# timmywanttolearn/distributed_model_parallel

Measured on AMD Instinct MI355X. Metric: images/sec (whole node) ResNet-50 DDP bf16, higher is better.
Workload: dtype bf16; 1 GPU; model=resnet50, device=cuda, global_batch=2048, per_gpu_batch=2048, image_size=224, parallelism=ddp1, single_rank_comm=False, ranks=1, rccl_ranks=1, launcher=single, optimizer=FlatSGD(fp32 master), sync_bn=False, channels_last=True, grad_comm=none(world_size=1), hip_graph=False, checkpoint_segments=0

## Files before the change

### csrc/api.h

```cpp
#pragma once

#include <ATen/ATen.h>
#include <c10/util/Optional.h>

#include <cstdint>
#include <string>
#include <vector>

namespace dmp {

bool attention_supported(int64_t S, int64_t head_dim);
void set_attention_variant(int fwd, int bwd);
std::vector<int64_t> get_attention_variant();
void set_attention_long_from(int64_t n);
int64_t get_attention_long_from();
std::vector<at::Tensor> attention_forward(const at::Tensor& qkv, int64_t B, int64_t S, int64_t H, double scale);
at::Tensor attention_backward(const at::Tensor& dout, const at::Tensor& qkv, const at::Tensor& o,
                              const at::Tensor& lse, int64_t B, int64_t S, int64_t H, double scale);

at::Tensor bn_local_moments(const at::Tensor& x, int64_t C);
std::vector<at::Tensor> bn_forward_apply(const at::Tensor& x, const at::Tensor& sums,
                                         const c10::optional<at::Tensor>& weight,
                                         const c10::optional<at::Tensor>& bias,
                                         const c10::optional<at::Tensor>& running_mean,
                                         const c10::optional<at::Tensor>& running_var,
                                         double momentum, double eps,
                                         const c10::optional<at::Tensor>& residual, bool relu,
                                         int64_t C,
                                         const c10::optional<at::Tensor>& num_batches_tracked,
                                         bool out_moments, double clip);
std::vector<at::Tensor> bn_eval_apply(const at::Tensor& x, const at::Tensor& running_mean,
                                      const at::Tensor& running_var,
                                      const c10::optional<at::Tensor>& weight,
                                      const c10::optional<at::Tensor>& bias, double eps,
                                      const c10::optional<at::Tensor>& residual, bool relu,
                                      int64_t C, double clip);
at::Tensor bn_backward_moments(const at::Tensor& dy, const at::Tensor& x,
                               const c10::optional<at::Tensor>& y, const at::Tensor& mean,
                               bool relu, int64_t C, const c10::optional<at::Tensor>& weight,
                               const c10::optional<at::Tensor>& bias,
                               const c10::optional<at::Tensor>& invstd, double clip);
at::Tensor bn_finalize(const at::Tensor& sums, const c10::optional<at::Tensor>& weight,
                       const c10::optional<at::Tensor>& bias,
                       const c10::optional<at::Tensor>& running_mean,
                       const c10::optional<at::Tensor>& running_var, double momentum, double eps,
                       int64_t C, const c10::optional<at::Tensor>& num_batches_tracked);
std::vector<at::Tensor> bn_backward_apply(const at::Tensor& dy, const at::Tensor& x,
                                          const c10::optional<at::Tensor>& y,
                                          const at::Tensor& sums, const at::Tensor& count,
                                          const c10::optional<at::Tensor>& weight,
                                          const at::Tensor& mean, const at::Tensor& invstd,
                                          bool training, bool relu, bool want_dres, int64_t C,
                                          const c10::optional<at::Tensor>& bias, double clip,
                                          const c10::optional<at::Tensor>& acc_weight,
                                          const c10::optional<at::Tensor>& acc_bias);
void set_bn_streaming(bool on);

bool bn_apply_gram_supported(int64_t C);
std::vector<at::Tensor> bn_forward_apply_gram(const at::Tensor& x, const at::Tensor& sums,
                                              const c10::optional<at::Tensor>& weight,
                                              const c10::optional<at::Tensor>& bias,
                                              const c10::optional<at::Tensor>& running_mean,
                                              const c10::optional<at::Tensor>& running_var, double momentum,
                                              double eps, int64_t C,
                                              const c10::optional<at::Tensor>& num_batches_tracked, double clip);
void set_bn_gram_blocks(int64_t n);

bool bn_fold_supported(int64_t cout, int64_t cin);
std::vector<at::Tensor> bn_fold_fwd(const at::Tensor& W, const at::Tensor& G, const at::Tensor& asums,
                                    const c10::optional<at::Tensor>& Wf);
std::vector<at::Tensor> bn_fold_fwd_finalize(const at::Tensor& W, const at::Tensor& G, const at::Tensor& asums,
                                             const c10::optional<at::Tensor>& Wf,
                                             const c10::optional<at::Tensor>& weight,
                                             const c10::optional<at::Tensor>& bias,
                                             const c10::optional<at::Tensor>& running_mean,
                                             const c10::optional<at::Tensor>& running_var, double momentum,
                                             double eps, const c10::optional<at::Tensor>& num_batches_tracked);
at::Tensor bn_fold_bwd_sums(const at::Tensor& D, const at::Tensor& W, const at::Tensor& sdz,
                            const at::Tensor& mean);
std::vector<at::Tensor> bn_fold_bwd_coef(const at::Tensor& sums, const at::Tensor& local, const at::Tensor& count,
                                         const at::Tensor& invstd, const at::Tensor& mean,
                                         const c10::optional<at::Tensor>& gamma, const at::Tensor& D,
                                         const at::Tensor& WG, const at::Tensor& s, const at::Tensor& W);
std::vector<at::Tensor> bn_fold_relu_mask(const at::Tensor& dy, const at::Tensor& y);
at::Tensor bn_fold_colsum(const at::Tensor& x, const std::vector<int64_t>& map);
std::vector<at::Tensor> bn_fold_scale_concat(const at::Tensor& W3, const at::Tensor& s3, const at::Tensor& t3,
                                             const at::Tensor& Wd, const at::Tensor& sd, const at::Tensor& td);
void set_fold_gemm(int mode);
int get_fold_gemm();

void multi_copy(const std::vector<at::Tensor>& srcs, const std::vector<at::Tensor>& dsts);
void multi_transpose(const std::vector<at::Tensor>& srcs, const std::vector<at::Tensor>& dsts,
                     const std::vector<int64_t>& taps);
void multi_cast_bf16_f32(const std::vector<at::Tensor>& srcs, const std::vector<at::Tensor>& dsts);
void reduce_add_into(const std::vector<at::Tensor>& inputs, at::Tensor& out);
void gather_slabs(const std::vector<at::Tensor>& inputs, at::Tensor& out, bool along_inner);
std::vector<std::vector<bool>> enable_peer_access(int64_t num_devices);

std::vector<at::Tensor> conv3x3_c128(const at::Tensor& x, const at::Tensor& wmat, bool moments);
bool conv3x3_c128_supported(int64_t c, int64_t h, int64_t w);
at::Tensor conv3x3_c128_dgrad_s2(const at::Tensor& dy, const at::Tensor& wt);

std::vector<at::Tensor> conv3x3_c64(const at::Tensor& x, const at::Tensor& wmat, bool moments);

std::vector<at::Tensor> dwconv3x3_forward(const at::Tensor& x, const at::Tensor& w, int64_t stride,
                                          bool moments);
at::Tensor dwconv3x3_dgrad(const at::Tensor& dy, const at::Tensor& w, int64_t stride, int64_t H,
                           int64_t W);
at::Tensor dwconv3x3_wgrad(const at::Tensor& dy, const at::Tensor& x, int64_t stride,
                           at::ScalarType out_dtype, const c10::optional<at::Tensor>& out);

std::vector<at::Tensor> gemm_nt(const at::Tensor& A, const at::Tensor& B,
                                const c10::optional<at::Tensor>& pro_scale,
                                const c10::optional<at::Tensor>& pro_shift, const std::string& mode,
                                const c10::optional<at::Tensor>& epi_scale,
                                const c10::optional<at::Tensor>& epi_shift,
                                const c10::optional<at::Tensor>& residual, bool relu,
                                const std::vector<int64_t>& a_map,
                                const std::vector<int64_t>& c_map,
                                const c10::optional<at::Tensor>& a2,
                                const std::vector<int64_t>& a2_map);
std::vector<at::Tensor> gemm_nt_bnbwd(const at::Tensor& A, const at::Tensor& B,
                                      const c10::optional<at::Tensor>& residual,
                                      const c10::optional<at::Tensor>& bn_x,
                                      const c10::optional<at::Tensor>& bn_y,
                                      const c10::optional<at::Tensor>& mean,
                                      const c10::optional<at::Tensor>& invstd,
                                      const c10::optional<at::Tensor>& weight,
                                      const c10::optional<at::Tensor>& bias,
                                      const std::vector<int64_t>& res_map,
                                      const c10::optional<at::Tensor>& a2,
                                      const c10::optional<at::Tensor>& ebias,
                                      const std::vector<int64_t>& a2_map);
at::Tensor gemm_tn(const at::Tensor& A, const at::Tensor& B, at::ScalarType out_dtype,
                   const std::vector<int64_t>& b_map, const c10::optional<at::Tensor>& pro_scale,
                   const c10::optional<at::Tensor>& pro_shift, bool a_mapped,
                   const c10::optional<at::Tensor>& out);
std::vector<at::Tensor> conv_nt(const at::Tensor& x, const at::Tensor& wmat, int64_t kh,
                                int64_t kw, int64_t stride, int64_t pad, int64_t ho, int64_t wo,
                                bool transposed, const c10::optional<at::Tensor>& pro_scale,
                                const c10::optional<at::Tensor>& pro_shift,
                                const std::string& mode,
                                const c10::optional<at::Tensor>& epi_scale,
                                const c10::optional<at::Tensor>& epi_shift,
                                const c10::optional<at::Tensor>& residual, bool relu,
                                int64_t kc);
at::Tensor conv_wgrad(const at::Tensor& dy, const at::Tensor& x, int64_t kh, int64_t kw,
                      int64_t stride, int64_t pad, int64_t ho, int64_t wo,
                      at::ScalarType out_dtype, int64_t kc, const c10::optional<at::Tensor>& out);
void set_gemm_tile(int64_t t);
void set_phase_dgrad(bool on);
void set_tn_wide(bool on);

at::Tensor space_to_depth2(const at::Tensor& x, int64_t pad, int64_t out_channels);
at::Tensor pad_channels16(const at::Tensor& x, int64_t pad, int64_t extra_w);

bool stem_halo_supported(int64_t hs, int64_t ws, int64_t ho, int64_t wo);
std::vector<at::Tensor> stem_halo_fwd(const at::Tensor& s, const at::Tensor& wm, int64_t ho, bool moments);
at::Tensor stem_halo_wgrad(const at::Tensor& dy, const at::Tensor& s, int64_t ho, at::ScalarType out_dtype);
std::vector<at::Tensor> stem_halo_wgrad_pool(const at::Tensor& dy, const at::Tensor& idx, const at::Tensor& y,
                                             const at::Tensor& s, const at::Tensor& scale, const at::Tensor& shift,
                                             const at::Tensor& mean, int64_t ho, int64_t pad);
at::Tensor stem_fold_finish(const at::Tensor& img, int64_t ho, int64_t wo, const at::Tensor& t_dz,
                            const at::Tensor& t_y, const at::Tensor& sums, const at::Tensor& cnt,
                            const at::Tensor& invstd, const c10::optional<at::Tensor>& weight, const at::Tensor& mean,
                            at::ScalarType out_dtype);

at::Tensor wgrad3x3(const at::Tensor& dy, const at::Tensor& x, int64_t stride);
bool wgrad3x3_supported(int64_t C, int64_t H, int64_t W, int64_t stride);
void set_wgrad3x3_waves(int64_t nw);

at::Tensor augment_batch(const at::Tensor& src, const at::Tensor& plan, int64_t out_h, int64_t out_w,
                         const std::vector<double>& mean, const std::vector<double>& std_, at::ScalarType dtype,
                         bool channels_last, bool no_resize);

at::Tensor batch_mix(const at::Tensor& x, const at::Tensor& perm, double lam, const std::vector<int64_t>& box);

at::Tensor gemm_xl(const at::Tensor& A, const at::Tensor& B, const std::string& mode,
                   const c10::optional<at::Tensor>& bias, const c10::optional<at::Tensor>& aux,
                   const c10::optional<at::Tensor>& residual, const c10::optional<at::Tensor>& out,
                   const c10::optional<at::Tensor>& row_scale = c10::nullopt, int64_t rows_per_sample = 0);
std::vector<at::Tensor> gemm_xl_dgelu_bgrad(const at::Tensor& A, const at::Tensor& B, const at::Tensor& aux);
std::vector<at::Tensor> gemm_xl_conv(const at::Tensor& A, const at::Tensor& B, const std::string& mode,
                                     const c10::optional<at::Tensor>& residual,
                                     const c10::optional<at::Tensor>& bn_x,
                                     const c10::optional<at::Tensor>& bn_y,
                                     const c10::optional<at::Tensor>& mean,
                                     const c10::optional<at::Tensor>& invstd,
                                     const c10::optional<at::Tensor>& weight,
                                     const c10::optional<at::Tensor>& bias,
                                     const std::vector<int64_t>& res_map,
                                     const c10::optional<at::Tensor>& a2,
                                     const c10::optional<at::Tensor>& ebias,
                                     const c10::optional<at::Tensor>& scale,
                                     const c10::optional<at::Tensor>& shift, bool relu,
                                     const std::vector<int64_t>& a2_map);
std::vector<at::Tensor> conv_xl(const at::Tensor& x, const at::Tensor& wmat, int64_t kh, int64_t kw,
                                int64_t stride, int64_t pad, int64_t ho, int64_t wo, const std::string& mode,
                                const c10::optional<at::Tensor>& residual, const c10::optional<at::Tensor>& bn_x,
                                const c10::optional<at::Tensor>& bn_y, const c10::optional<at::Tensor>& mean,
                                const c10::optional<at::Tensor>& invstd, const c10::optional<at::Tensor>& weight,
                                const c10::optional<at::Tensor>& bias);
at::Tensor conv_xl_dgrad_s2(const at::Tensor& dy, const std::vector<at::Tensor>& wph, int64_t hi, int64_t wi);
void set_gemm_xl_bn(int bn, int pipe, int group_m);
int get_gemm_xl_pipe();
void set_gemm_xl_x2(int mode);
int get_gemm_xl_x2();
void set_gemm_xl_bm(int bm);
int get_gemm_xl_bm(int64_t M, int64_t N, int64_t K);
void set_gemm_xl_trace(const c10::optional<at::Tensor>& buf);
void set_gemm_xl_trim_heavy(bool on);

at::Tensor gemm_tn_xl(const at::Tensor& A, const at::Tensor& B, at::ScalarType out_dtype,
                      const c10::optional<at::Tensor>& out);
at::Tensor gram_strided_xl(const at::Tensor& x, int64_t stride, int64_t ho, int64_t wo);
bool gram_strided_xl_supported(int64_t nb, int64_t cin, int64_t hi, int64_t wi, int64_t ho, int64_t wo);
at::Tensor conv_wgrad_xl(const at::Tensor& dy, const at::Tensor& x, int64_t kh, int64_t kw, int64_t stride,
                         int64_t pad, int64_t ho, int64_t wo, at::ScalarType out_dtype,
                         const c10::optional<at::Tensor>& out);
void set_tn_xl_rounds(int r);
void set_tn_narrow(bool on);

bool colsum_supported(int64_t N);
at::Tensor bias_grad(const at::Tensor& dy, at::ScalarType out_dtype);
std::vector<at::Tensor> gelu_bwd_bias_grad(const at::Tensor& dy, const at::Tensor& h, at::ScalarType out_dtype);
std::vector<at::Tensor> rowscale_bias_grad(const at::Tensor& dy, const at::Tensor& row_scale, int64_t rows_per_sample,
                                           at::ScalarType out_dtype);

std::vector<at::Tensor> cross_entropy_fwd(const at::Tensor& x, const at::Tensor& target,
                                          int64_t ignore_index, double scale,
                                          const c10::optional<at::Tensor>& acc, double label_smoothing,
                                          const c10::optional<at::Tensor>& target_b, double lam);
at::Tensor cross_entropy_bwd(const at::Tensor& grad, const at::Tensor& x, const at::Tensor& target,
                             const at::Tensor& lse, const at::Tensor& stats, int64_t ignore_index,
                             double label_smoothing, const c10::optional<at::Tensor>& target_b, double lam);
std::vector<at::Tensor> layernorm_forward(const at::Tensor& x, const c10::optional<at::Tensor>& w,
                                          const c10::optional<at::Tensor>& b, int64_t D,
                                          double eps);
std::vector<at::Tensor> layernorm_backward(const at::Tensor& dy, const at::Tensor& x,
                                           const c10::optional<at::Tensor>& w,
                                           const at::Tensor& mean, const at::Tensor& rstd,
                                           int64_t D, at::ScalarType param_dtype,
                                           const c10::optional<at::Tensor>& dres);
bool layernorm_supported(int64_t D);

void flat_sumsq_partials(const at::Tensor& grad, at::Tensor& partials_row);
void adamw_prepare(const c10::optional<at::Tensor>& partials, at::Tensor& hyper, at::Tensor& step,
                   double max_norm, double beta1, double beta2);
void adamw_flat_step(const c10::optional<at::Tensor>& master, at::Tensor& exp_avg, at::Tensor& exp_avg_sq,
                     const at::Tensor& grad, at::Tensor& param,
                     const c10::optional<at::Tensor>& decay_mask, const at::Tensor& hyper, double lr,
                     double beta1, double beta2, double eps, double weight_decay,
                     const c10::optional<at::Tensor>& ema, double ema_decay);
int64_t adamw_grid_cap();

void lars_norm_partials(const c10::optional<at::Tensor>& master, const at::Tensor& grad,
                        const at::Tensor& param, const at::Tensor& items, at::Tensor& partials);
void lars_trust(const at::Tensor& partials, const at::Tensor& tensors, at::Tensor& coef,
                double trust_coefficient, double weight_decay, double eps);
void lars_flat_step(const c10::optional<at::Tensor>& master, at::Tensor& mom, const at::Tensor& grad,
                    at::Tensor& param, const at::Tensor& items, const at::Tensor& coef, double lr,
                    double momentum, const c10::optional<at::Tensor>& ema, double ema_decay);
int64_t lars_chunk_elems();
int64_t lars_fold_threads();

void sgd_flat_step(const c10::optional<at::Tensor>& master, const at::Tensor& mom,
                   const at::Tensor& grad, const at::Tensor& param, double lr, double wd,
                   double momentum, double dampening, bool nesterov, double grad_scale,
                   bool first_step, const c10::optional<at::Tensor>& ema, double ema_decay);

std::vector<at::Tensor> maxpool2d_forward(const at::Tensor& x, int64_t k, int64_t s, int64_t p);
at::Tensor maxpool2d_backward(const at::Tensor& dy, const at::Tensor& idx, int64_t H, int64_t W,
                              int64_t k, int64_t s, int64_t p);
at::Tensor global_avgpool_backward(const at::Tensor& g, int64_t H, int64_t W);
std::vector<at::Tensor> maxpool2d_bn_forward(const at::Tensor& x, const at::Tensor& scale,
                                             const at::Tensor& shift, int64_t k, int64_t s, int64_t p);
std::vector<at::Tensor> maxpool2d_bn_backward(const at::Tensor& dy, const at::Tensor& idx, const at::Tensor& x,
                                              const at::Tensor& scale, const at::Tensor& shift,
                                              const at::Tensor& mean, int64_t k, int64_t s, int64_t p);
void set_pool_generic(bool on);

}
```

### csrc/bindings.cpp

```cpp
#include <cmath>
#include <torch/extension.h>
#include <torch/csrc/autograd/variable.h>

#include "api.h"
#include "comm/rccl_comm.h"
#include "ddp/reducer.h"
#include "dp/parallel_apply.h"

namespace py = pybind11;

PYBIND11_MODULE(TORCH_EXTENSION_NAME, m) {
  m.doc() = "MI355X-native runtime: RCCL communicator, DDP reducer, HIP kernels (gfx950)";

  m.def("bn_local_moments", &dmp::bn_local_moments,
        py::call_guard<py::gil_scoped_release>());
  m.def("bn_forward_apply", &dmp::bn_forward_apply, py::arg("x"), py::arg("sums"), py::arg("weight"),
        py::arg("bias"), py::arg("running_mean"), py::arg("running_var"), py::arg("momentum"),
        py::arg("eps"), py::arg("residual"), py::arg("relu"), py::arg("C"),
        py::arg("num_batches_tracked") = py::none(), py::arg("out_moments") = false,
        py::arg("clip") = INFINITY,
        py::call_guard<py::gil_scoped_release>());
  m.def("bn_forward_apply_gram", &dmp::bn_forward_apply_gram, py::arg("x"), py::arg("sums"), py::arg("weight"),
        py::arg("bias"), py::arg("running_mean"), py::arg("running_var"), py::arg("momentum"), py::arg("eps"),
        py::arg("C"), py::arg("num_batches_tracked") = py::none(), py::arg("clip") = INFINITY,
        "training-mode BN + ReLU apply that also returns the column moments and the fp32 Gram of its output",
        py::call_guard<py::gil_scoped_release>());
  m.def("bn_apply_gram_supported", &dmp::bn_apply_gram_supported);
  m.def("set_bn_gram_blocks", &dmp::set_bn_gram_blocks);
  m.def("bn_eval_apply", &dmp::bn_eval_apply, py::arg("x"), py::arg("running_mean"),
        py::arg("running_var"), py::arg("weight"), py::arg("bias"), py::arg("eps"), py::arg("residual"),
        py::arg("relu"), py::arg("C"), py::arg("clip") = INFINITY,
        py::call_guard<py::gil_scoped_release>());
  m.def("bn_finalize", &dmp::bn_finalize, py::arg("sums"), py::arg("weight"), py::arg("bias"),
        py::arg("running_mean"), py::arg("running_var"), py::arg("momentum"), py::arg("eps"),
        py::arg("C"), py::arg("num_batches_tracked") = py::none(),
        py::call_guard<py::gil_scoped_release>());
  m.def("bn_backward_moments", &dmp::bn_backward_moments, py::arg("dy"), py::arg("x"), py::arg("y"),
        py::arg("mean"), py::arg("relu"), py::arg("C"), py::arg("weight") = py::none(),
        py::arg("bias") = py::none(), py::arg("invstd") = py::none(), py::arg("clip") = INFINITY,
        py::call_guard<py::gil_scoped_release>());
  m.def("bn_backward_apply", &dmp::bn_backward_apply, py::arg("dy"), py::arg("x"), py::arg("y"),
        py::arg("sums"), py::arg("count"), py::arg("weight"), py::arg("mean"), py::arg("invstd"),
        py::arg("training"), py::arg("relu"), py::arg("want_dres"), py::arg("C"),
        py::arg("bias") = py::none(), py::arg("clip") = INFINITY, py::arg("acc_weight") = py::none(),
        py::arg("acc_bias") = py::none(),
        py::call_guard<py::gil_scoped_release>());

  m.def("gemm_nt", &dmp::gemm_nt, py::arg("A"), py::arg("B"), py::arg("pro_scale") = py::none(),
        py::arg("pro_shift") = py::none(), py::arg("mode") = "store",
        py::arg("epi_scale") = py::none(), py::arg("epi_shift") = py::none(),
        py::arg("residual") = py::none(), py::arg("relu") = false,
        py::arg("a_map") = std::vector<int64_t>{}, py::arg("c_map") = std::vector<int64_t>{},
        py::arg("a2") = py::none(), py::arg("a2_map") = std::vector<int64_t>{},
        py::call_guard<py::gil_scoped_release>());

  m.def("cross_entropy_fwd", &dmp::cross_entropy_fwd, py::arg("x"), py::arg("target"),
        py::arg("ignore_index") = -100, py::arg("scale") = 1.0, py::arg("acc") = py::none(),
        py::arg("label_smoothing") = 0.0, py::arg("target_b") = py::none(), py::arg("lam") = 1.0,
        "scale * mean softmax cross-entropy; acc (fp64 [3]) += (loss, top-1 correct, top-5 correct); "
        "label_smoothing and a second label target_b weighted 1 - lam give the soft-target loss",
        py::call_guard<py::gil_scoped_release>());
  m.def("cross_entropy_bwd", &dmp::cross_entropy_bwd, py::arg("grad"), py::arg("x"), py::arg("target"),
        py::arg("lse"), py::arg("stats"), py::arg("ignore_index") = -100, py::arg("label_smoothing") = 0.0,
        py::arg("target_b") = py::none(), py::arg("lam") = 1.0, py::call_guard<py::gil_scoped_release>());
  m.def("batch_mix", &dmp::batch_mix, py::arg("x"), py::arg("perm"), py::arg("lam"),
        py::arg("box") = std::vector<int64_t>{},
        "mixup (empty box): lam * x[i] + (1 - lam) * x[perm[i]]; CutMix (box = [y0, y1, x0, x1]): "
        "x[perm[i]] inside the box, x[i] outside; channels-last bf16 / fp32, out of place",
        py::call_guard<py::gil_scoped_release>());
  m.def("augment_batch", &dmp::augment_batch, py::arg("src"), py::arg("plan"), py::arg("out_h"), py::arg("out_w"),
        py::arg("mean"), py::arg("std"), py::arg("dtype"), py::arg("channels_last") = true, py::arg("no_resize") = false,
        "uint8 NHWC batch -> [B, C, out_h, out_w] bf16 / fp32: per-sample crop box plan[i] = (x0, y0, cw, ch, flip) "
        "(zero padding outside the image, bilinear resize when the box is not out_h x out_w), flip, /255, "
        "mean / std normalisation, cast and layout in one launch; no_resize: every box is out_h x out_w (the crop-only kernel; "
        "other rows come out NaN)",
        py::call_guard<py::gil_scoped_release>());
  m.def("gemm_nt_bnbwd", &dmp::gemm_nt_bnbwd, py::arg("A"), py::arg("B"), py::arg("residual"),
        py::arg("bn_x"), py::arg("bn_y"), py::arg("mean"), py::arg("invstd"), py::arg("weight"),
        py::arg("bias"), py::arg("res_map") = std::vector<int64_t>{}, py::arg("a2") = py::none(),
        py::arg("ebias") = py::none(), py::arg("a2_map") = std::vector<int64_t>{},
        py::call_guard<py::gil_scoped_release>());

  m.def("gemm_tn", &dmp::gemm_tn, py::arg("A"), py::arg("B"), py::arg("out_dtype"),
        py::arg("b_map") = std::vector<int64_t>{}, py::arg("pro_scale") = py::none(),
        py::arg("pro_shift") = py::none(), py::arg("a_mapped") = false, py::arg("out") = py::none(),
        "C = A^T B (weight gradient); b_map reads B's rows through a strided map, a_mapped A's too (Gram of a "
        "sample); out: add into this gradient instead of returning a new tensor",
        py::call_guard<py::gil_scoped_release>());

  m.def("set_tn_wide", &dmp::set_tn_wide, py::arg("on"),
        "128 x 256 TN tiles for deep weight gradients (default on)");
  m.def("set_phase_dgrad", &dmp::set_phase_dgrad, py::arg("on"),
        "strided implicit-GEMM data gradients as stride-phase launches (default on)");
  m.def("set_gemm_tile", &dmp::set_gemm_tile,
        "debug: force the NT GEMM tile variant (-1 auto, 0 256x64, 1 128x64, 2 128x128, "
        "3 128x64/4x1, 4 64x128, 5 64x64)");

  m.def("conv_nt", &dmp::conv_nt, py::arg("x"), py::arg("wmat"), py::arg("kh"), py::arg("kw"),
        py::arg("stride"), py::arg("pad"), py::arg("ho"), py::arg("wo"),
        py::arg("transposed") = false, py::arg("pro_scale") = py::none(),
        py::arg("pro_shift") = py::none(), py::arg("mode") = "store",
        py::arg("epi_scale") = py::none(), py::arg("epi_shift") = py::none(),
        py::arg("residual") = py::none(), py::arg("relu") = false, py::arg("kc") = 0,
        py::call_guard<py::gil_scoped_release>());
  m.def("conv_wgrad", &dmp::conv_wgrad, py::arg("dy"), py::arg("x"), py::arg("kh"), py::arg("kw"),
        py::arg("stride"), py::arg("pad"), py::arg("ho"), py::arg("wo"), py::arg("out_dtype"),
        py::arg("kc") = 0, py::arg("out") = py::none(),
        py::call_guard<py::gil_scoped_release>());
  m.def("maxpool2d_bn_forward", &dmp::maxpool2d_bn_forward, py::arg("x"), py::arg("scale"),
        py::arg("shift"), py::arg("k"), py::arg("s"), py::arg("p"),
        py::call_guard<py::gil_scoped_release>());
  m.def("maxpool2d_bn_backward", &dmp::maxpool2d_bn_backward, py::arg("dy"), py::arg("idx"), py::arg("x"),
        py::arg("scale"), py::arg("shift"), py::arg("mean"), py::arg("k"), py::arg("s"), py::arg("p"),
        py::call_guard<py::gil_scoped_release>());
  m.def("pad_channels16", &dmp::pad_channels16, py::arg("x"), py::arg("pad"), py::arg("extra_w") = 0,
        py::call_guard<py::gil_scoped_release>());
  m.def("space_to_depth2", &dmp::space_to_depth2, py::arg("x"), py::arg("pad"), py::arg("out_channels") = 16,
        py::call_guard<py::gil_scoped_release>());

  m.def("gemm_xl", &dmp::gemm_xl, py::arg("A"), py::arg("B"), py::arg("mode") = "store",
        py::arg("bias") = py::none(), py::arg("aux") = py::none(),
        py::arg("residual") = py::none(), py::arg("out") = py::none(), py::kw_only(),
        py::arg("row_scale") = py::none(), py::arg("rows_per_sample") = 0,
        py::call_guard<py::gil_scoped_release>());
  m.def("conv_xl", &dmp::conv_xl, py::arg("x"), py::arg("wmat"), py::arg("kh"), py::arg("kw"),
        py::arg("stride"), py::arg("pad"), py::arg("ho"), py::arg("wo"), py::arg("mode") = "moments",
        py::arg("residual") = py::none(), py::arg("bn_x") = py::none(), py::arg("bn_y") = py::none(),
        py::arg("mean") = py::none(), py::arg("invstd") = py::none(), py::arg("weight") = py::none(),
        py::arg("bias") = py::none(),
        "Implicit-GEMM conv (NHWC gather) on the 256x256 ping-pong MFMA kernel with conv epilogues",
        py::call_guard<py::gil_scoped_release>());
  m.def("stem_halo_supported", &dmp::stem_halo_supported);
  m.def("stem_halo_fwd", &dmp::stem_halo_fwd, py::arg("s"), py::arg("wm"), py::arg("ho"), py::arg("moments") = false,
        "ResNet stem (s2d 4x4 conv, 16 -> 64 ch, Wo = 112) forward: halo-tiled, weights in VGPRs",
        py::call_guard<py::gil_scoped_release>());
  m.def("stem_fold_finish", &dmp::stem_fold_finish, py::arg("img"), py::arg("ho"), py::arg("wo"), py::arg("t_dz"),
        py::arg("t_y"), py::arg("sums"), py::arg("cnt"), py::arg("invstd"), py::arg("weight"), py::arg("mean"),
        py::arg("out_dtype"),
        "folded stem weight gradient: BN-backward coefficients, the 16 window sums of the batch-summed "
        "space-to-depth image, and al t_dz + be t_y + cc cols in one launch",
        py::call_guard<py::gil_scoped_release>());
  m.def("stem_halo_wgrad", &dmp::stem_halo_wgrad, py::arg("dy"), py::arg("s"), py::arg("ho"), py::arg("out_dtype"),
        "ResNet stem weight gradient [64, 256]: halo-tiled, dW in VGPRs",
        py::call_guard<py::gil_scoped_release>());
  m.def("stem_halo_wgrad_pool", &dmp::stem_halo_wgrad_pool, py::arg("dy"), py::arg("idx"), py::arg("y"), py::arg("s"),
        py::arg("scale"), py::arg("shift"), py::arg("mean"), py::arg("ho"), py::arg("pad"),
        "ResNet stem folded backward: (dz^T P, y^T P, BN-backward sums) with the pool / ReLU backward formed in LDS",
        py::call_guard<py::gil_scoped_release>());
  m.def("wgrad3x3", &dmp::wgrad3x3, py::arg("dy"), py::arg("x"), py::arg("stride") = 1,
        "dW [C, C, 3, 3] (channels_last) of a 3x3/s1/p1 conv: persistent halo-tiled MFMA kernel",
        py::call_guard<py::gil_scoped_release>());
  m.def("wgrad3x3_supported", &dmp::wgrad3x3_supported, py::arg("C"), py::arg("Ho"), py::arg("Wo"),
        py::arg("stride") = 1);
  m.def("set_wgrad3x3_waves", &dmp::set_wgrad3x3_waves);
  m.def("conv3x3_c64", &dmp::conv3x3_c64, py::arg("x"), py::arg("wmat"), py::arg("moments") = false,
        "3x3/s1/p1 64->64-channel conv (W = 56) on the persistent halo-tiled MFMA kernel; "
        "returns (y [N*H*W, 64], fp64 moments [129] or empty)",
        py::call_guard<py::gil_scoped_release>());
  m.def("conv3x3_c128", &dmp::conv3x3_c128, py::arg("x"), py::arg("wmat"), py::arg("moments") = false,
        "3x3/s1/p1 128->128-channel conv (W = 28, H % 4 == 0) on the persistent halo-tiled MFMA kernel "
        "(Cout split over grid halves, K split over wave pairs); returns (y [N*H*W, 128], fp64 moments [257] or empty)",
        py::call_guard<py::gil_scoped_release>());
  m.def("conv3x3_c128_dgrad_s2", &dmp::conv3x3_c128_dgrad_s2, py::arg("dy"), py::arg("wt"),
        "data gradient of a 3x3/s2/p1 128->128 conv (dy 28 wide) as its four stride phases on the halo kernel; "
        "wt = W.permute(1, 2, 3, 0) as [128, 1152]; returns dx [N*2H*56, 128]",
        py::call_guard<py::gil_scoped_release>());
  m.def("conv3x3_c128_supported", &dmp::conv3x3_c128_supported, py::arg("C"), py::arg("H"), py::arg("W"));
  m.def("conv_xl_dgrad_s2", &dmp::conv_xl_dgrad_s2, py::arg("dy"), py::arg("wph"), py::arg("hi"), py::arg("wi"),
        "data gradient of a 3x3/s2/p1 conv as four stride-phase implicit GEMMs on the ping-pong kernel; "
        "returns dx [N*hi*wi, Cin]",
        py::call_guard<py::gil_scoped_release>());
  m.def("set_bn_streaming", &dmp::set_bn_streaming, py::arg("on"),
        "A/B: non-temporal streaming in the BN apply passes over > 256 MB tensors (default on)");
  m.def("set_pool_generic", &dmp::set_pool_generic, py::arg("on"),
        "A/B: route every max-pool geometry through the runtime-k kernels (default off)");
  m.def("set_tn_xl_rounds", &dmp::set_tn_xl_rounds, py::arg("rounds"));
  m.def("set_gemm_xl_trim_heavy", &dmp::set_gemm_xl_trim_heavy, py::arg("on"),
        "A/B: trimmed (192..240-row) tiles for the PIPE-10 heavy-epilogue GEMMs at any K (default on)");
  m.def("set_tn_narrow", &dmp::set_tn_narrow, py::arg("on"),
        "A/B: 4-wave weight-gradient tiles of 64 / 128 on an output side that narrow (default on)");
  m.def("gemm_tn_xl", &dmp::gemm_tn_xl, py::arg("A"), py::arg("B"), py::arg("out_dtype"), py::arg("out") = py::none(),
        "A^T B (weight gradient) on the ping-pong MFMA schedule, split over M",
        py::call_guard<py::gil_scoped_release>());
  m.def("gram_strided_xl", &dmp::gram_strided_xl, py::arg("x"), py::arg("stride"), py::arg("ho"), py::arg("wo"),
        "fp32 Gram x_s^T x_s of the stride-s sample of an NHWC bf16 input (4-wave TN kernel, both operands gathered)",
        py::call_guard<py::gil_scoped_release>());
  m.def("gram_strided_xl_supported", &dmp::gram_strided_xl_supported);
  m.def("conv_wgrad_xl", &dmp::conv_wgrad_xl, py::arg("dy"), py::arg("x"), py::arg("kh"), py::arg("kw"),
        py::arg("stride"), py::arg("pad"), py::arg("ho"), py::arg("wo"), py::arg("out_dtype"),
        py::arg("out") = py::none(),
        "kh x kw conv weight gradient (tap gather) on the ping-pong TN kernel; Cin % 256 == 0",
        py::call_guard<py::gil_scoped_release>());
  m.def("gemm_xl_dgelu_bgrad", &dmp::gemm_xl_dgelu_bgrad, py::arg("A"), py::arg("B"), py::arg("aux"),
        py::call_guard<py::gil_scoped_release>());
  m.def("gemm_xl_conv", &dmp::gemm_xl_conv, py::arg("A"), py::arg("B"), py::arg("mode"),
        py::arg("residual") = py::none(), py::arg("bn_x") = py::none(), py::arg("bn_y") = py::none(),
        py::arg("mean") = py::none(), py::arg("invstd") = py::none(), py::arg("weight") = py::none(),
        py::arg("bias") = py::none(), py::arg("res_map") = std::vector<int64_t>{},
        py::arg("a2") = py::none(), py::arg("ebias") = py::none(), py::arg("scale") = py::none(),
        py::arg("shift") = py::none(), py::arg("relu") = false, py::arg("a2_map") = std::vector<int64_t>{},
        "wide 1x1-conv GEMM with conv epilogues: moments | add | bnbwd | affine (scale, shift, residual, relu); "
        "a2: second A source concatenated along K; ebias: bnbwd per-column constant",
        py::call_guard<py::gil_scoped_release>());
  m.def("get_gemm_xl_pipe", &dmp::get_gemm_xl_pipe);
  m.def("set_gemm_xl_x2", &dmp::set_gemm_xl_x2, py::arg("mode"),
        "conv-epilogue GEMMs on the two-blocks-per-CU 256x128 kernel: 0 off, 1 where N % 256 != 0, 2 always");
  m.def("get_gemm_xl_x2", &dmp::get_gemm_xl_x2);
  m.def("set_gemm_xl_bm", &dmp::set_gemm_xl_bm, py::arg("bm"),
        "256x256 ping-pong GEMMs: rows per tile (0 auto: trimmed to fill whole rounds when K >= 768; "
        "-1 always 256; 192..240 forced)");
  m.def("set_gemm_xl_trace", &dmp::set_gemm_xl_trace, py::arg("buf") = py::none(),
        "diagnostics: 256x256 ping-pong GEMM launches record per-block phase timestamps into buf "
        "(int64 [blocks * 8]: entry, operands landed, main loop done, epilogue done, HW_ID, XCC_ID); None = off");
  m.def("get_gemm_xl_bm", &dmp::get_gemm_xl_bm, py::arg("M"), py::arg("N"), py::arg("K"),
        "rows per tile the ping-pong GEMM would take for this shape");
  m.def("set_gemm_xl_bn", &dmp::set_gemm_xl_bn, py::arg("bn"), py::arg("pipe") = -1, py::arg("group_m") = 0,
        "debug: force the gemm_xl N tile (0 auto, 128, 256) and main loop (0, 1, 10, 11; -1 default)");

  m.def("bn_fold_supported", &dmp::bn_fold_supported, py::arg("cout"), py::arg("cin"));
  m.def("bn_fold_fwd_finalize", &dmp::bn_fold_fwd_finalize, py::arg("W"), py::arg("G"), py::arg("asums"),
        py::arg("Wf"), py::arg("weight"), py::arg("bias"), py::arg("running_mean"), py::arg("running_var"),
        py::arg("momentum"), py::arg("eps"), py::arg("num_batches_tracked"),
        "bn_fold_fwd + the BN finalize of its moments in one launch: (sums, WG, coef[4, Cout])");
  m.def("bn_fold_fwd", &dmp::bn_fold_fwd, py::arg("W"), py::arg("G"), py::arg("asums"), py::arg("Wf") = py::none(),
        "(sums fp64 [2Cout+1], WG fp32 [Cout, Cin]) of y = a W^T from G = a^T a and colsum(a)",
        py::call_guard<py::gil_scoped_release>());
  m.def("bn_fold_bwd_sums", &dmp::bn_fold_bwd_sums, py::arg("D"), py::arg("W"), py::arg("sdz"), py::arg("mean"),
        "local fp64 [2Cout] = (sum dz, sum dz*(y - mean)) from D = dz^T a",
        py::call_guard<py::gil_scoped_release>());
  m.def("bn_fold_bwd_coef", &dmp::bn_fold_bwd_coef, py::arg("sums"), py::arg("local"), py::arg("count"),
        py::arg("invstd"), py::arg("mean"), py::arg("gamma"), py::arg("D"), py::arg("WG"), py::arg("s"),
        py::arg("W"), "(dW, dgamma, dbeta, Bm = [(al o W)^T | W^T diag(be) W], ebias = c^T W)",
        py::call_guard<py::gil_scoped_release>());

  m.def("bn_fold_relu_mask", &dmp::bn_fold_relu_mask, py::arg("dy"), py::arg("y"),
        py::call_guard<py::gil_scoped_release>());
  m.def("bn_fold_colsum", &dmp::bn_fold_colsum, py::arg("x"), py::arg("map") = std::vector<int64_t>{},
        "fp64 [2C+1] (colsum, colsum of squares, rows) of x's rows sampled through a strided map",
        py::call_guard<py::gil_scoped_release>());
  m.def("bn_fold_scale_concat", &dmp::bn_fold_scale_concat, py::arg("W3"), py::arg("s3"), py::arg("t3"),
        py::arg("Wd"), py::arg("sd"), py::arg("td"), "([s3 o W3 | sd o Wd] bf16, t3 + td)",
        py::call_guard<py::gil_scoped_release>());

  m.def("attention_supported", &dmp::attention_supported);
  m.def("set_fold_gemm", &dmp::set_fold_gemm, py::arg("mode"),
        "BN-fold coefficient products: 0 fused VALU kernels, 1 library fp32 GEMMs (default), 2 tiled kernel");
  m.def("get_fold_gemm", &dmp::get_fold_gemm);
  m.def("get_attention_variant", &dmp::get_attention_variant);
  m.def("set_attention_variant", &dmp::set_attention_variant, py::arg("fwd"), py::arg("bwd") = 1,
        "attention kernels: fwd 0 = one workgroup per (batch, head), 1 = persistent with next-head prefetch, "
        "2 = 8-wave per head; bwd 0 = per head, 1 = persistent with prefetch.  Selects among the S <= 256 "
        "kernels only: the streamed long-sequence kernels (set_attention_long_from) have one variant each");
  m.def("get_attention_long_from", &dmp::get_attention_long_from);
  m.def("set_attention_long_from", &dmp::set_attention_long_from, py::arg("n"),
        "sequences of n tokens or more run the streamed long-sequence attention kernels (default 257: "
        "everything the whole-sequence-in-LDS kernels cannot hold; 1 = always, for A/B runs and tests)");
  m.def("attention_forward", &dmp::attention_forward, py::arg("qkv"), py::arg("B"), py::arg("S"),
        py::arg("H"), py::arg("scale"),
        py::call_guard<py::gil_scoped_release>());
  m.def("attention_backward", &dmp::attention_backward, py::arg("dout"), py::arg("qkv"), py::arg("o"),
        py::arg("lse"), py::arg("B"), py::arg("S"), py::arg("H"), py::arg("scale"),
        py::call_guard<py::gil_scoped_release>());

  m.def("colsum_supported", &dmp::colsum_supported);
  m.def("bias_grad", &dmp::bias_grad, py::arg("dy"), py::arg("out_dtype"),
        py::call_guard<py::gil_scoped_release>());
  m.def("gelu_bwd_bias_grad", &dmp::gelu_bwd_bias_grad, py::arg("dy"), py::arg("h"), py::arg("out_dtype"),
        py::call_guard<py::gil_scoped_release>());
  m.def("rowscale_bias_grad", &dmp::rowscale_bias_grad, py::arg("dy"), py::arg("row_scale"),
        py::arg("rows_per_sample"), py::arg("out_dtype"), py::call_guard<py::gil_scoped_release>());

  m.def("layernorm_forward", &dmp::layernorm_forward,
        py::call_guard<py::gil_scoped_release>());
  m.def("layernorm_backward", &dmp::layernorm_backward, py::arg("dy"), py::arg("x"), py::arg("w"),
        py::arg("mean"), py::arg("rstd"), py::arg("D"), py::arg("param_dtype"),
        py::arg("dres") = py::none(),
        py::call_guard<py::gil_scoped_release>());
  m.def("layernorm_supported", &dmp::layernorm_supported);

  m.def("maxpool2d_forward", &dmp::maxpool2d_forward,
        py::call_guard<py::gil_scoped_release>());
  m.def("maxpool2d_backward", &dmp::maxpool2d_backward,
        py::call_guard<py::gil_scoped_release>());
  m.def("global_avgpool_backward", &dmp::global_avgpool_backward,
        py::call_guard<py::gil_scoped_release>());

  m.def("dwconv3x3_forward", &dmp::dwconv3x3_forward, py::arg("x"), py::arg("w"),
        py::arg("stride"), py::arg("moments") = false,
        py::call_guard<py::gil_scoped_release>());
  m.def("dwconv3x3_dgrad", &dmp::dwconv3x3_dgrad,
        py::call_guard<py::gil_scoped_release>());
  m.def("dwconv3x3_wgrad", &dmp::dwconv3x3_wgrad, py::arg("dy"), py::arg("x"), py::arg("stride"),
        py::arg("out_dtype"), py::arg("out") = py::none(),
        py::call_guard<py::gil_scoped_release>());

  m.def("sgd_flat_step", &dmp::sgd_flat_step, py::arg("master"), py::arg("mom"), py::arg("grad"),
        py::arg("param"), py::arg("lr"), py::arg("wd"), py::arg("momentum"), py::arg("dampening"),
        py::arg("nesterov"), py::arg("grad_scale"), py::arg("first_step"), py::arg("ema") = py::none(),
        py::arg("ema_decay") = 0.0,
        py::call_guard<py::gil_scoped_release>());
  m.def("flat_sumsq_partials", &dmp::flat_sumsq_partials, py::arg("grad"), py::arg("partials_row"),
        "partials_row[b] = block b's sum of squares of the flat gradient (fixed order, no atomics)",
        py::call_guard<py::gil_scoped_release>());
  m.def("adamw_prepare", &dmp::adamw_prepare, py::arg("partials"), py::arg("hyper"), py::arg("step"),
        py::arg("max_norm"), py::arg("beta1"), py::arg("beta2"),
        "step += 1; hyper = {1 - beta1^step, 1 - beta2^step, gradient norm, clip coefficient}",
        py::call_guard<py::gil_scoped_release>());
  m.def("adamw_flat_step", &dmp::adamw_flat_step, py::arg("master"), py::arg("exp_avg"),
        py::arg("exp_avg_sq"), py::arg("grad"), py::arg("param"), py::arg("decay_mask"), py::arg("hyper"),
        py::arg("lr"), py::arg("beta1"), py::arg("beta2"), py::arg("eps"), py::arg("weight_decay"),
        py::arg("ema") = py::none(), py::arg("ema_decay") = 0.0,
        py::call_guard<py::gil_scoped_release>());
  m.def("adamw_grid_cap", &dmp::adamw_grid_cap);
  m.def("lars_norm_partials", &dmp::lars_norm_partials, py::arg("master"), py::arg("grad"), py::arg("param"),
        py::arg("items"), py::arg("partials"),
        "partials[i] = {sum g^2, sum w^2} over work item i (fixed order, no atomics)",
        py::call_guard<py::gil_scoped_release>());
  m.def("lars_trust", &dmp::lars_trust, py::arg("partials"), py::arg("tensors"), py::arg("coef"),
        py::arg("trust_coefficient"), py::arg("weight_decay"), py::arg("eps"),
        "coef[t] = {trust ratio, weight decay, |w|, |g|} of tensor t; {1, 0, ..} for an excluded tensor",
        py::call_guard<py::gil_scoped_release>());
  m.def("lars_flat_step", &dmp::lars_flat_step, py::arg("master"), py::arg("mom"), py::arg("grad"),
        py::arg("param"), py::arg("items"), py::arg("coef"), py::arg("lr"), py::arg("momentum"),
        py::arg("ema") = py::none(), py::arg("ema_decay") = 0.0,
        py::call_guard<py::gil_scoped_release>());
  m.def("lars_chunk_elems", &dmp::lars_chunk_elems);
  m.def("lars_fold_threads", &dmp::lars_fold_threads);

  m.def("multi_copy", &dmp::multi_copy,
        py::call_guard<py::gil_scoped_release>());
  m.def("multi_cast_bf16_f32", &dmp::multi_cast_bf16_f32, py::arg("srcs"), py::arg("dsts"),
        "dst[i] (fp32) = src[i] (bf16) for contiguous tensors, up to 64 per launch",
        py::call_guard<py::gil_scoped_release>());
  m.def("multi_transpose", &dmp::multi_transpose, py::arg("srcs"), py::arg("dsts"),
        py::arg("taps") = std::vector<int64_t>{},
        "dst[i] = src[i]^T for contiguous 2-byte matrices, up to 64 per launch; taps[i] = T (-T: "
        "flipped) transposes [R, T*C] -> [C, T*R] tap by tap",
        py::call_guard<py::gil_scoped_release>());
  m.def("reduce_add_into", &dmp::reduce_add_into,
        py::call_guard<py::gil_scoped_release>());
  m.def("gather_slabs", &dmp::gather_slabs,
        py::call_guard<py::gil_scoped_release>());
  m.def("enable_peer_access", &dmp::enable_peer_access);

  py::class_<dmp::RcclComm, std::shared_ptr<dmp::RcclComm>>(m, "RcclComm")
      .def(py::init<const std::string&, int64_t, int64_t, int64_t, bool>(), py::arg("unique_id"),
           py::arg("nranks"), py::arg("rank"), py::arg("device"), py::arg("high_priority") = false,
           py::call_guard<py::gil_scoped_release>())
      .def("set_inline", &dmp::RcclComm::set_inline)
      .def("is_inline", &dmp::RcclComm::is_inline)
      .def_static("new_unique_id", [] { return py::bytes(dmp::RcclComm::new_unique_id()); })
      .def_property_readonly("rank", &dmp::RcclComm::rank)
      .def_property_readonly("size", &dmp::RcclComm::size)
      .def_property_readonly("device", &dmp::RcclComm::device)
      .def("all_reduce", &dmp::RcclComm::all_reduce, py::arg("tensor"), py::arg("op") = "sum",
           py::arg("on_current_stream") = false, py::call_guard<py::gil_scoped_release>())
      .def("all_reduce_coalesced", &dmp::RcclComm::all_reduce_coalesced, py::arg("tensors"),
           py::arg("op") = "sum", py::call_guard<py::gil_scoped_release>())
      .def("broadcast", &dmp::RcclComm::broadcast, py::call_guard<py::gil_scoped_release>())
      .def("reduce", &dmp::RcclComm::reduce, py::arg("tensor"), py::arg("root"),
           py::arg("op") = "sum", py::call_guard<py::gil_scoped_release>())
      .def("all_gather", &dmp::RcclComm::all_gather, py::call_guard<py::gil_scoped_release>())
      .def("reduce_scatter", &dmp::RcclComm::reduce_scatter, py::arg("out"), py::arg("inp"),
           py::arg("op") = "sum", py::call_guard<py::gil_scoped_release>())
      .def("all_to_all", &dmp::RcclComm::all_to_all, py::call_guard<py::gil_scoped_release>())
      .def("send", &dmp::RcclComm::send, py::call_guard<py::gil_scoped_release>())
      .def("recv", &dmp::RcclComm::recv, py::call_guard<py::gil_scoped_release>())
      .def("batch_p2p", &dmp::RcclComm::batch_p2p, py::call_guard<py::gil_scoped_release>())
      .def("wait", &dmp::RcclComm::wait, py::call_guard<py::gil_scoped_release>())
      .def("synchronize", &dmp::RcclComm::synchronize, py::call_guard<py::gil_scoped_release>())
      .def("stream_handle",
           [](const dmp::RcclComm& c) { return reinterpret_cast<uintptr_t>(c.stream()); });

  py::class_<dmp::ParallelApply, std::shared_ptr<dmp::ParallelApply>>(m, "ParallelApply")
      .def(py::init<>())
      .def("apply", &dmp::ParallelApply::apply, py::arg("modules"), py::arg("inputs"),
           py::arg("kwargs"), py::arg("devices"), py::arg("streams") = std::vector<int64_t>{})
      .def("num_workers", &dmp::ParallelApply::num_workers)
      .def("last_times", &dmp::ParallelApply::last_times);

  py::class_<dmp::ReduceBackend, std::shared_ptr<dmp::ReduceBackend>>(m, "ReduceBackend");
  py::class_<dmp::RcclReduceBackend, dmp::ReduceBackend, std::shared_ptr<dmp::RcclReduceBackend>>(
      m, "RcclReduceBackend")
      .def(py::init<std::shared_ptr<dmp::RcclComm>, double, int64_t, bool>(), py::arg("comm"),
           py::arg("postscale") = 1.0, py::arg("debug_delay_cycles") = 0, py::arg("fp32_accum") = false)
      .def("set_timing", &dmp::RcclReduceBackend::set_timing, py::arg("on"))
      .def("last_timing", &dmp::RcclReduceBackend::last_timing,
           "[ready->done ms per bucket..., collective ms per bucket..., exposed tail ms] of the last backward",
           py::call_guard<py::gil_scoped_release>());
  py::class_<dmp::NullReduceBackend, dmp::ReduceBackend, std::shared_ptr<dmp::NullReduceBackend>>(
      m, "NullReduceBackend")
      .def(py::init<>());
  py::class_<dmp::PyReduceBackend, dmp::ReduceBackend, std::shared_ptr<dmp::PyReduceBackend>>(
      m, "PyReduceBackend")
      .def(py::init<py::object>());

  py::class_<dmp::Reducer, std::shared_ptr<dmp::Reducer>>(m, "Reducer")
      .def(py::init<std::vector<at::Tensor>, std::vector<std::vector<int64_t>>,
                    std::shared_ptr<dmp::ReduceBackend>, bool>(),
           py::arg("params"), py::arg("buckets"), py::arg("backend"), py::arg("find_unused"))
      .def("prepare_for_backward", &dmp::Reducer::prepare_for_backward,
           py::call_guard<py::gil_scoped_release>())
      .def("disarm", &dmp::Reducer::disarm)
      .def("rebuild", &dmp::Reducer::rebuild, py::call_guard<py::gil_scoped_release>())
      .def("buckets", &dmp::Reducer::buckets)
      .def("ready_order", &dmp::Reducer::ready_order)
      .def("group_flats", &dmp::Reducer::group_flats)
      .def("layout", &dmp::Reducer::layout)
      .def("grad_views", &dmp::Reducer::grad_views)
      .def("unused_params", &dmp::Reducer::unused_params)
      .def("num_launched", &dmp::Reducer::num_launched)
      .def("set_backend", &dmp::Reducer::set_backend)
      .def("zero_grad", &dmp::Reducer::zero_grad, py::call_guard<py::gil_scoped_release>());

  m.def("compute_bucket_assignment", &dmp::compute_bucket_assignment, py::arg("params"),
        py::arg("cap_bytes"), py::arg("first_cap_bytes"));
  m.def("grad_accumulator_stream", [](const at::Tensor& t) -> int64_t {
    auto acc = torch::autograd::impl::try_get_grad_accumulator(t);
    if (!acc) return -1;
    auto s = acc->stream();
    return s.has_value() ? (int64_t)s->id() : -2;
  });
}
```

### csrc/conv/conv3x3_c128.hip

```cpp
#include <torch/extension.h>
#include <ATen/hip/HIPContext.h>
#include "../api.h"
#include "../common.h"
#include "../launch.h"

namespace dmp {
namespace {

using bf16 = __bf16;
using lptr_t = __attribute__((address_space(3))) void*;

constexpr int CI = 128, CO = 128, CB = 64;
constexpr int W = 28, R = 4;
constexpr int NT = 256;
constexpr int OUT_PIX = R * W;
constexpr int MF = OUT_PIX / 16;
constexpr int MF_LO = 4;
constexpr int KSTEPS = 9 * 64 / 32;

template <bool PH>
struct Geo {
  static constexpr int HR = PH ? R + 1 : R + 2, HC = PH ? W + 1 : W + 2;
  static constexpr int OFF = PH ? 0 : 1;
  static constexpr int PIX = HR * HC;
  static constexpr int DMA_INSTR = (PIX * (CI / 8) + 63) / 64;
  static constexpr int DMA_PER_WAVE = (DMA_INSTR + 3) / 4;
  static constexpr int BUF = DMA_PER_WAVE * 4 * 1024;
  static constexpr int SCR_OFF = 2 * BUF;
  static constexpr int STAGE_OFF = SCR_OFF + 2 * MF * 2 * 1024;
  static constexpr int MRED_OFF = STAGE_OFF + OUT_PIX * CB * 2;
  static constexpr int SMEM = MRED_OFF + 2 * CB * 4;
  static constexpr int MIN_STORES = PH ? 12 : 3;
  static_assert(SMEM <= 160 * 1024, "LDS budget");
};

__device__ __attribute__((aligned(16))) uint32_t g_c128_zero[4];

__device__ __forceinline__ int hkey(int q) { return (q & 7) << 1; }
__device__ __forceinline__ int stage_key(int p) { return ((p >> 2) & 3) << 1; }

__device__ __forceinline__ void glds16(const void* g, char* lds) {
  const uint32_t l = (uint32_t)(uintptr_t)(lptr_t)lds;
  asm volatile("s_mov_b32 m0, %0\n\ts_nop 0\n\tglobal_load_lds_dwordx4 %1, off"
               :: "s"(__builtin_amdgcn_readfirstlane(l)), "v"(g) : "memory", "m0");
}
template <int N>
__device__ __forceinline__ void vmcnt() {
  asm volatile("s_waitcnt vmcnt(%0)" ::"n"(N) : "memory");
}
__device__ __forceinline__ void raw_barrier() {
  asm volatile("" ::: "memory");
  __builtin_amdgcn_s_barrier();
  asm volatile("" ::: "memory");
}

template <bool PH>
struct Slots {
  int pk[Geo<PH>::DMA_PER_WAVE];
  uint32_t xok = 0;
};

template <bool PH>
__device__ __forceinline__ Slots<PH> make_slots(int wave, int lane) {
  using G = Geo<PH>;
  Slots<PH> s;
#pragma unroll
  for (int i = 0; i < G::DMA_PER_WAVE; ++i) {
    const int ins = wave * G::DMA_PER_WAVE + i;
    const int g = ins * 64 + lane;
    const int q = g >> 4;
    const int c = (g & 15) ^ hkey(q);
    const int hy = q / G::HC, hx = q - hy * G::HC, ix = hx - G::OFF;
    s.pk[i] = (((hy - G::OFF) * W + ix) * CI + c * 8) * 8 + min(hy, 7);
    if (q < G::PIX && ins < G::DMA_INSTR && ix >= 0 && ix < W) s.xok |= 1u << i;
  }
  return s;
}

template <bool PH>
__device__ __forceinline__ void halo_issue(const bf16* __restrict__ x, char* buf, int tile, int H, int tpi,
                                           int wave, const Slots<PH>& s) {
  using G = Geo<PH>;
  const int n = tile / tpi;
  const int r0 = (tile - n * tpi) * R;
  const bf16* base = x + ((int64_t)n * H + r0) * W * CI;
  const int rlo = G::OFF - r0, rhi = H - r0 + G::OFF;
#pragma unroll
  for (int i = 0; i < G::DMA_PER_WAVE; ++i) {
    const int ins = wave * G::DMA_PER_WAVE + i;
    const int hy = s.pk[i] & 7;
    const bool ok = ((s.xok >> i) & 1u) && hy >= rlo && hy < rhi;
    const void* src = ok ? (const void*)(base + (s.pk[i] >> 3)) : (const void*)g_c128_zero;
    if (ins < G::DMA_INSTR) glds16(src, buf + ins * 1024);
  }
}

__host__ __device__ constexpr int ph_k(int p, int i) { return p == 0 ? 1 : (i == 0 ? 2 : 0); }
__host__ __device__ constexpr int ph_a(int p, int i) { return p == 0 ? 0 : i; }

template <bool PH, int PY, int PX>
__device__ __forceinline__ void sweep(f32x4 (&acc)[MF][2], const bf16x8 (&bw)[2][KSTEPS], const char* hb,
                                      const int (&qb)[MF], const uint32_t (&kt)[MF], int lchunk) {
  using G = Geo<PH>;
  constexpr int NTY = PH ? (PY ? 2 : 1) : 3, NTX = PH ? (PX ? 2 : 1) : 3;
  constexpr int KS = 2 * NTY * NTX;
  bf16x8 a[2][MF];
  auto load_step = [&](int s, bf16x8 (&dst)[MF]) __attribute__((always_inline)) {
    const int t = s >> 1, ty = t / NTX, tx = t - ty * NTX;
    const int oy = PH ? ph_a(PY, ty) : ty, ox = PH ? ph_a(PX, tx) : tx;
    const int o = oy * G::HC + ox;
#pragma unroll
    for (int f = 0; f < MF; ++f) {
      const int key = (int)((kt[f] >> (4 * (o & 7))) & 15u);
      const int ch = (lchunk + 4 * (s & 1)) ^ key;
      dst[f] = *reinterpret_cast<const bf16x8*>(hb + qb[f] + o * (CI * 2) + (ch << 4));
    }
  };
  load_step(0, a[0]);
#pragma unroll
  for (int s = 0; s < KS; ++s) {
    if (s + 1 < KS) load_step(s + 1, a[(s + 1) & 1]);
    const int t = s >> 1, ty = t / NTX, tx = t - ty * NTX;
    const int ky = PH ? ph_k(PY, ty) : ty, kx = PH ? ph_k(PX, tx) : tx;
    const int ws = (ky * 3 + kx) * 2 + (s & 1);
#pragma unroll
    for (int f = 0; f < MF; ++f)
#pragma unroll
      for (int nf = 0; nf < 2; ++nf)
        acc[f][nf] = __builtin_amdgcn_mfma_f32_16x16x32_bf16(a[s & 1][f], bw[nf][ws], acc[f][nf], 0, 0, 0);
    if (s + 1 < KS) {
#pragma unroll
      for (int f = 0; f < MF; ++f) {
        __builtin_amdgcn_sched_group_barrier(0x100, 1, 0);
        __builtin_amdgcn_sched_group_barrier(0x008, 1, 0);
      }
      __builtin_amdgcn_sched_group_barrier(0x008, MF, 0);
    }
    __builtin_amdgcn_sched_barrier(0);
  }
}

template <int F0, int F1>
__device__ __forceinline__ void send_frags(const f32x4 (&acc)[MF][2], f32x4* scr, int wn, int lane) {
#pragma unroll
  for (int f = F0; f < F1; ++f)
#pragma unroll
    for (int nf = 0; nf < 2; ++nf) scr[((wn * MF + f) * 2 + nf) * 64 + lane] = acc[f][nf];
}

template <int F0, int F1>
__device__ __forceinline__ void finish_frags(const f32x4 (&acc)[MF][2], const f32x4* scr, bf16* ostage, int wn,
                                             int lane, int l15, int lh) {
#pragma unroll
  for (int f = F0; f < F1; ++f)
#pragma unroll
    for (int nf = 0; nf < 2; ++nf) {
      const f32x4 o = scr[((wn * MF + f) * 2 + nf) * 64 + lane];
#pragma unroll
      for (int i = 0; i < 4; ++i) {
        const int p = f * 16 + 4 * lh + i;
        const int ch = (4 * wn + 2 * nf + (l15 >> 3)) ^ stage_key(p);
        ostage[p * CB + ch * 8 + (l15 & 7)] = (bf16)(acc[f][nf][i] + o[i]);
      }
    }
}

__device__ __forceinline__ void exchange_to_stage(const f32x4 (&acc)[MF][2], f32x4* scr, bf16* ostage, int wkh,
                                                  int wn, int lane, int l15, int lh) {
  if (wkh == 0) send_frags<MF_LO, MF>(acc, scr, wn, lane);
  else send_frags<0, MF_LO>(acc, scr, wn, lane);
  __syncthreads();
  if (wkh == 0) finish_frags<0, MF_LO>(acc, scr, ostage, wn, lane, l15, lh);
  else finish_frags<MF_LO, MF>(acc, scr, ostage, wn, lane, l15, lh);
  __syncthreads();
}

template <bool MOM, bool PH>
__global__ __launch_bounds__(NT, 1) void conv3x3_c128_kernel(
    const bf16* __restrict__ x, const bf16* __restrict__ wk, bf16* __restrict__ y, float* __restrict__ part,
    double* zsums, int H, int tiles) {
  using G = Geo<PH>;
  __shared__ __attribute__((aligned(1024))) char smem[G::SMEM];
  f32x4* scr = reinterpret_cast<f32x4*>(smem + G::SCR_OFF);
  bf16* ostage = reinterpret_cast<bf16*>(smem + G::STAGE_OFF);
  float* mred = reinterpret_cast<float*>(smem + G::MRED_OFF);
  const int lane = threadIdx.x & 63, wave = threadIdx.x >> 6;
  const int wkh = wave & 1, wn = wave >> 1;
  const int l15 = lane & 15, lh = lane >> 4;
  const int half = (int)gridDim.x >> 1;
  const int cb = (int)blockIdx.x >= half ? 1 : 0;
  const int rb = (int)blockIdx.x - cb * half;
  const int tpi = H / R;
  if constexpr (MOM) {
    zero_moments(zsums, 2 * CO);
    if (threadIdx.x < 2 * CB) mred[threadIdx.x] = 0.f;
  }
  const int t_begin = (int)((int64_t)tiles * rb / half);
  const int t_end = (int)((int64_t)tiles * (rb + 1) / half);
  const Slots<PH> sl = make_slots<PH>(wave, lane);
  if (t_begin < t_end) halo_issue<PH>(x, smem, t_begin, H, tpi, wave, sl);

  bf16x8 bw[2][KSTEPS];
#pragma unroll
  for (int nf = 0; nf < 2; ++nf) {
    const bf16* wrow = wk + (int64_t)(CB * cb + 32 * wn + 16 * nf + l15) * (9 * CI) + 64 * wkh + 8 * lh;
#pragma unroll
    for (int s = 0; s < KSTEPS; ++s)
      bw[nf][s] = *reinterpret_cast<const bf16x8*>(wrow + (s >> 1) * CI + 32 * (s & 1));
  }
  int qb[MF];
  uint32_t kt[MF];
  const int lchunk = 8 * wkh + lh;
#pragma unroll
  for (int f = 0; f < MF; ++f) {
    const int p = f * 16 + l15;
    const int oy = p / W, ox = p - oy * W;
    const int q = oy * G::HC + ox;
    qb[f] = q * (CI * 2);
    uint32_t t = 0;
#pragma unroll
    for (int i = 0; i < 8; ++i) t |= (uint32_t)hkey(q + i) << (4 * i);
    kt[f] = t;
  }

  float s8[8], q8[8];
#pragma unroll
  for (int j = 0; j < 8; ++j) s8[j] = q8[j] = 0.f;
  int cur = 0;
  bool stored_prev = false;
  for (int t = t_begin; t < t_end; ++t) {
#pragma unroll
    for (int f = 0; f < MF; ++f) asm volatile("" : "+v"(kt[f]), "+v"(qb[f]));
    if (stored_prev) vmcnt<G::MIN_STORES>();
    else vmcnt<0>();
    raw_barrier();
    if (t + 1 < t_end) halo_issue<PH>(x, smem + (cur ^ 1) * G::BUF, t + 1, H, tpi, wave, sl);
    const char* hb = smem + cur * G::BUF;
    const int n = t / tpi;
    const int r0 = (t - n * tpi) * R;

    auto store_stage = [&](int py, int px) __attribute__((always_inline)) {
      for (int i = threadIdx.x; i < OUT_PIX * 8; i += NT) {
        const int sp = i >> 3;
        const bf16x8 v = *reinterpret_cast<const bf16x8*>(ostage + sp * CB + (((i & 7) ^ stage_key(sp)) << 3));
        int64_t pix;
        if constexpr (PH) {
          const int m = sp / W, q = sp - m * W;
          pix = ((int64_t)n * (2 * H) + 2 * (r0 + m) + py) * (2 * W) + 2 * q + px;
        } else {
          pix = ((int64_t)n * H + r0) * W + sp;
        }
        *reinterpret_cast<bf16x8*>(y + pix * CO + CB * cb + (i & 7) * 8) = v;
        if constexpr (MOM)
#pragma unroll
          for (int j = 0; j < 8; ++j) {
            const float fv = (float)v[j];
            s8[j] += fv;
            q8[j] = fmaf(fv, fv, q8[j]);
          }
      }
    };
    auto phase = [&](auto pyc, auto pxc) __attribute__((always_inline)) {
      constexpr int PY = decltype(pyc)::value, PX = decltype(pxc)::value;
      f32x4 acc[MF][2];
#pragma unroll
      for (int f = 0; f < MF; ++f) acc[f][0] = acc[f][1] = f32x4{0.f, 0.f, 0.f, 0.f};
      sweep<PH, PY, PX>(acc, bw, hb, qb, kt, lchunk);
      exchange_to_stage(acc, scr, ostage, wkh, wn, lane, l15, lh);
      store_stage(PY < 0 ? 0 : PY, PX < 0 ? 0 : PX);
    };
    using I0 = std::integral_constant<int, 0>;
    using I1 = std::integral_constant<int, 1>;
    using IN = std::integral_constant<int, -1>;
    if constexpr (PH) {
      phase(I0{}, I0{});
      phase(I0{}, I1{});
      phase(I1{}, I0{});
      phase(I1{}, I1{});
    } else {
      phase(IN{}, IN{});
    }
    stored_prev = true;
    cur ^= 1;
  }

  if constexpr (MOM) {
#pragma unroll
    for (int j = 0; j < 8; ++j)
#pragma unroll
      for (int off = 8; off < 64; off <<= 1) {
        s8[j] += __shfl_xor(s8[j], off, 64);
        q8[j] += __shfl_xor(q8[j], off, 64);
      }
    if (lane < 8)
#pragma unroll
      for (int j = 0; j < 8; ++j) {
        atomicAdd(&mred[8 * lane + j], s8[j]);
        atomicAdd(&mred[CB + 8 * lane + j], q8[j]);
      }
    __syncthreads();
    if (threadIdx.x < 2 * CB) {
      const int mo = threadIdx.x / CB, ch = threadIdx.x % CB;
      part[((int64_t)mo * half + rb) * CO + CB * cb + ch] = mred[mo * CB + ch];
    }
  }
}

int grid_half(int tiles) {
  int dev = 0, cus = 256;
  DMP_HIP_CHECK(hipGetDevice(&dev));
  DMP_HIP_CHECK(hipDeviceGetAttribute(&cus, hipDeviceAttributeMultiprocessorCount, dev));
  return std::max(1, std::min(tiles, cus / 2));
}

void check_wmat(const at::Tensor& wmat, const char* who) {
  TORCH_CHECK(wmat.scalar_type() == at::kBFloat16 && wmat.is_contiguous() && wmat.dim() == 2 &&
                  wmat.size(0) == CO && wmat.size(1) == 9 * CI, who, ": wmat must be contiguous [128, 1152] bf16");
}

}

bool conv3x3_c128_supported(int64_t c, int64_t h, int64_t w) {
  return c == CI && w == W && h > 0 && h % R == 0;
}

std::vector<at::Tensor> conv3x3_c128(const at::Tensor& x, const at::Tensor& wmat, bool moments) {
  TORCH_CHECK(x.is_cuda() && x.scalar_type() == at::kBFloat16 && x.dim() == 4, "conv3x3_c128: bf16 NCHW-shaped x");
  TORCH_CHECK(conv3x3_c128_supported(x.size(1), x.size(2), x.size(3)) &&
                  x.is_contiguous(at::MemoryFormat::ChannelsLast),
              "conv3x3_c128: x must be [N, 128, H % 4 == 0, 28] channels_last");
  check_wmat(wmat, "conv3x3_c128");
  TORCH_CHECK(wmat.device() == x.device(), "conv3x3_c128: device mismatch");
  const int64_t n = x.size(0), H = x.size(2);
  const int64_t tiles64 = n * (H / R);
  TORCH_CHECK(tiles64 < (1 << 30), "conv3x3_c128: too many tiles");
  const int tiles = (int)tiles64;
  auto y = at::empty({n * H * W, CO}, x.options());
  if (tiles == 0) return {y, at::zeros({moments ? 2 * CO + 1 : 0}, x.options().dtype(at::kDouble))};
  auto stream = at::hip::getCurrentHIPStream();
  const int half = grid_half(tiles);
  const int grid = 2 * half;
  at::Tensor mom;
  if (moments) {
    mom = at::empty({2 * CO + 1}, x.options().dtype(at::kDouble));
    auto part = at::empty({2, half, CO}, x.options().dtype(at::kFloat));
    hipLaunchKernelGGL((conv3x3_c128_kernel<true, false>), dim3(grid), dim3(NT), 0, stream,
                       reinterpret_cast<const bf16*>(x.data_ptr()), reinterpret_cast<const bf16*>(wmat.data_ptr()),
                       reinterpret_cast<bf16*>(y.data_ptr()), part.data_ptr<float>(),
                       moments_zero_target(mom.data_ptr<double>(), half), (int)H, tiles);
    bn_reduce_partials_launch(part.data_ptr<float>(), half, CO, mom.data_ptr<double>(), (double)(n * H * W),
                              stream);
  } else {
    mom = at::empty({0}, x.options().dtype(at::kDouble));
    hipLaunchKernelGGL((conv3x3_c128_kernel<false, false>), dim3(grid), dim3(NT), 0, stream,
                       reinterpret_cast<const bf16*>(x.data_ptr()), reinterpret_cast<const bf16*>(wmat.data_ptr()),
                       reinterpret_cast<bf16*>(y.data_ptr()), nullptr, nullptr, (int)H, tiles);
  }
  DMP_HIP_CHECK(hipGetLastError());
  return {y, mom};
}

at::Tensor conv3x3_c128_dgrad_s2(const at::Tensor& dy, const at::Tensor& wt) {
  TORCH_CHECK(dy.is_cuda() && dy.scalar_type() == at::kBFloat16 && dy.dim() == 4,
              "conv3x3_c128_dgrad_s2: bf16 NCHW-shaped dy");
  TORCH_CHECK(conv3x3_c128_supported(dy.size(1), dy.size(2), dy.size(3)) &&
                  dy.is_contiguous(at::MemoryFormat::ChannelsLast),
              "conv3x3_c128_dgrad_s2: dy must be [N, 128, H % 4 == 0, 28] channels_last");
  check_wmat(wt, "conv3x3_c128_dgrad_s2");
  TORCH_CHECK(wt.device() == dy.device(), "conv3x3_c128_dgrad_s2: device mismatch");
  const int64_t n = dy.size(0), H = dy.size(2);
  const int64_t tiles64 = n * (H / R);
  TORCH_CHECK(tiles64 < (1 << 30) && n * 4 * H * W < (1LL << 31), "conv3x3_c128_dgrad_s2: too large");
  const int tiles = (int)tiles64;
  auto dx = at::empty({n * 4 * H * W, CI}, dy.options());
  if (tiles == 0) return dx;
  auto stream = at::hip::getCurrentHIPStream();
  const int half = grid_half(tiles);
  hipLaunchKernelGGL((conv3x3_c128_kernel<false, true>), dim3(2 * half), dim3(NT), 0, stream,
                     reinterpret_cast<const bf16*>(dy.data_ptr()), reinterpret_cast<const bf16*>(wt.data_ptr()),
                     reinterpret_cast<bf16*>(dx.data_ptr()), nullptr, nullptr, (int)H, tiles);
  DMP_HIP_CHECK(hipGetLastError());
  return dx;
}

}
```

### csrc/conv/conv3x3_halo.hip

```cpp
#include <cstdlib>
#include <torch/extension.h>
#include <ATen/hip/HIPContext.h>
#include "../api.h"
#include "../common.h"
#include "../launch.h"

namespace dmp {
namespace {

using bf16 = __bf16;
using gptr_t = const __attribute__((address_space(1))) void*;
using lptr_t = __attribute__((address_space(3))) void*;

constexpr int C64 = 64;
constexpr int KSTEPS = 9 * C64 / 32;

__device__ __attribute__((aligned(16))) uint32_t g_halo_zero[4];

template <int W, int R, int NW>
struct HaloGeo {
  static constexpr int NT = 64 * NW;
  static constexpr int NFW = 8 / NW;
  static constexpr int HW2 = W + 2;
  static constexpr int PIX = (R + 2) * HW2;
  static constexpr int DMA_INSTR = (PIX * 8 + 63) / 64;
  static constexpr int DMA_PER_WAVE = (DMA_INSTR + NW - 1) / NW;
  static constexpr int BUF_BYTES = DMA_PER_WAVE * NW * 1024;
  static constexpr int OUT_PIX = R * W;
  static constexpr int SMEM_BYTES = 2 * BUF_BYTES + OUT_PIX * 64 * 2 + 2 * 64 * 4;
  static constexpr int MFRAG = OUT_PIX / 16;
  static constexpr int MF_WAVE = MFRAG / 2;
  static constexpr int STORES_PER_THREAD = OUT_PIX * 8 / NT;
  static constexpr bool STORES_EXACT = OUT_PIX * 8 % NT == 0;
  static_assert(NW == 4 || NW == 8, "4 waves (2 x 32 channels each) or 8 (1 x 16)");
  static_assert(OUT_PIX % 32 == 0, "R*W must split into 2 x 16-row fragments");
};

constexpr uint32_t kHaloKeys = 0x31165572u;
__device__ __forceinline__ int halo_key(int q) { return (0x31165572u >> (4 * (q & 7))) & 7; }

__device__ __forceinline__ int stage_key(int p) { return (p >> 1) & 7; }

__device__ __forceinline__ void glds16(const void* g, char* lds) {
  const uint32_t l = (uint32_t)(uintptr_t)(lptr_t)lds;
  asm volatile("s_mov_b32 m0, %0\n\ts_nop 0\n\tglobal_load_lds_dwordx4 %1, off"
               :: "s"(__builtin_amdgcn_readfirstlane(l)), "v"(g) : "memory", "m0");
}

template <int N>
__device__ __forceinline__ void vmcnt() {
  asm volatile("s_waitcnt vmcnt(%0)" ::"n"(N) : "memory");
}
__device__ __forceinline__ void raw_barrier() {
  asm volatile("" ::: "memory");
  __builtin_amdgcn_s_barrier();
  asm volatile("" ::: "memory");
}

template <int W, int R, int NW>
struct HaloSlots {
  int pk[HaloGeo<W, R, NW>::DMA_PER_WAVE];
  uint32_t xok = 0;
};

template <int W, int R, int NW>
__device__ __forceinline__ HaloSlots<W, R, NW> halo_slots(int wave, int lane) {
  using G = HaloGeo<W, R, NW>;
  HaloSlots<W, R, NW> hs;
#pragma unroll
  for (int i = 0; i < G::DMA_PER_WAVE; ++i) {
    const int ins = wave * G::DMA_PER_WAVE + i;
    const int g = ins * 64 + lane;
    const int q = g >> 3;
    const int c = (g & 7) ^ halo_key(q);
    const int hy = q / G::HW2, hx = q - hy * G::HW2;
    const int ix = hx - 1;
    hs.pk[i] = (((hy - 1) * W + ix) * C64 + c * 8) * 8 + min(hy, 7);
    if (q < G::PIX && ins < G::DMA_INSTR && ix >= 0 && ix < W) hs.xok |= 1u << i;
  }
  return hs;
}

template <int W, int R, int NW>
__device__ __forceinline__ void halo_issue(const bf16* __restrict__ x, char* buf, int tile, int H,
                                           int tiles_per_img, int wave, int lane,
                                           const HaloSlots<W, R, NW>& hs) {
  using G = HaloGeo<W, R, NW>;
  const int n = tile / tiles_per_img;
  const int r0 = (tile - n * tiles_per_img) * R;
  const bf16* base = x + ((int64_t)n * H + r0) * W * C64;
  const int rlo = 1 - r0, rhi = H - r0 + 1;
#pragma unroll
  for (int i = 0; i < G::DMA_PER_WAVE; ++i) {
    const int ins = wave * G::DMA_PER_WAVE + i;
    const int hy = hs.pk[i] & 7;
    const bool ok = ((hs.xok >> i) & 1u) && hy >= rlo && hy < rhi;
    const void* src = ok ? (const void*)(base + (hs.pk[i] >> 3)) : (const void*)g_halo_zero;
    if (ins < G::DMA_INSTR)
      glds16(src, buf + ins * 1024);
  }
}

template <int W, int R, int NW, bool MOM>
__global__ __launch_bounds__(64 * NW, 1) void conv3x3_c64_kernel(
    const bf16* __restrict__ x, const bf16* __restrict__ wk, bf16* __restrict__ y, float* __restrict__ part,
    double* zsums, int H, int tiles, int tiles_per_img) {
  using G = HaloGeo<W, R, NW>;
  constexpr int NFW = G::NFW;
  __shared__ __attribute__((aligned(1024))) char smem[G::SMEM_BYTES];
  bf16* ostage = reinterpret_cast<bf16*>(smem + 2 * G::BUF_BYTES);
  float* mred = reinterpret_cast<float*>(smem + 2 * G::BUF_BYTES + G::OUT_PIX * C64 * 2);
  const int lane = threadIdx.x & 63, wave = threadIdx.x >> 6;
  const int wm = wave & 1, wn = wave >> 1;
  const int l15 = lane & 15, lh = lane >> 4;
  if constexpr (MOM) {
    zero_moments(zsums, 2 * C64);
    if (threadIdx.x < 2 * C64) mred[threadIdx.x] = 0.f;
  }

  const int t_begin = (int)((int64_t)tiles * blockIdx.x / gridDim.x);
  const int t_end = (int)((int64_t)tiles * (blockIdx.x + 1) / gridDim.x);
  const HaloSlots<W, R, NW> hs = halo_slots<W, R, NW>(wave, lane);
  if (t_begin < t_end) halo_issue<W, R, NW>(x, smem, t_begin, H, tiles_per_img, wave, lane, hs);

  bf16x8 bw[NFW][KSTEPS];
#pragma unroll
  for (int nf = 0; nf < NFW; ++nf) {
    const bf16* wrow = wk + (int64_t)(16 * (NFW * wn + nf) + l15) * (9 * C64) + 8 * lh;
#pragma unroll
    for (int s = 0; s < KSTEPS; ++s) bw[nf][s] = *reinterpret_cast<const bf16x8*>(wrow + 32 * s);
  }
  int qb[G::MF_WAVE];
  uint32_t kt[G::MF_WAVE];
#pragma unroll
  for (int f = 0; f < G::MF_WAVE; ++f) {
    const int p = (wm * G::MF_WAVE + f) * 16 + l15;
    const int oy = p / W, ox = p - oy * W;
    const int q = oy * G::HW2 + ox;
    qb[f] = q * 128;
    const uint32_t r = 4u * (uint32_t)(q & 7);
    const uint32_t rot = r == 0 ? kHaloKeys : (kHaloKeys >> r) | (kHaloKeys << (32u - r));
    kt[f] = rot ^ (0x11111111u * (uint32_t)lh);
  }

  float s8[8], q8[8];
#pragma unroll
  for (int j = 0; j < 8; ++j) s8[j] = q8[j] = 0.f;
  int cur = 0;
  bool full_prev = false;
  for (int t = t_begin; t < t_end; ++t) {
#pragma unroll
    for (int f = 0; f < G::MF_WAVE; ++f) asm volatile("" : "+v"(kt[f]), "+v"(qb[f]));
    if constexpr (G::STORES_EXACT) {
      if (full_prev) vmcnt<G::STORES_PER_THREAD>();
      else vmcnt<0>();
    } else {
      vmcnt<0>();
    }
    raw_barrier();
    if (t + 1 < t_end) halo_issue<W, R, NW>(x, smem + (cur ^ 1) * G::BUF_BYTES, t + 1, H, tiles_per_img, wave, lane, hs);
    const char* hb = smem + cur * G::BUF_BYTES;

    f32x4 acc[G::MF_WAVE][NFW];
#pragma unroll
    for (int f = 0; f < G::MF_WAVE; ++f)
#pragma unroll
      for (int nf = 0; nf < NFW; ++nf) acc[f][nf] = f32x4{0.f, 0.f, 0.f, 0.f};

    bf16x8 a[2][G::MF_WAVE];
    auto load_step = [&](int s, bf16x8 (&dst)[G::MF_WAVE]) {
      const int tap = s >> 1, kh = tap / 3, kw = tap - 3 * (tap / 3);
      const int o = kh * G::HW2 + kw;
#pragma unroll
      for (int f = 0; f < G::MF_WAVE; ++f) {
        const uint32_t ch = ((kt[f] >> (4 * (o & 7))) & 7u) ^ (uint32_t)((s & 1) * 4);
        dst[f] = *reinterpret_cast<const bf16x8*>(hb + qb[f] + o * 128 + (ch << 4));
      }
    };
    load_step(0, a[0]);
#pragma unroll
    for (int s = 0; s < KSTEPS; ++s) {
      if (s + 1 < KSTEPS) load_step(s + 1, a[(s + 1) & 1]);
#pragma unroll
      for (int f = 0; f < G::MF_WAVE; ++f)
#pragma unroll
        for (int nf = 0; nf < NFW; ++nf)
          acc[f][nf] = __builtin_amdgcn_mfma_f32_16x16x32_bf16(bw[nf][s], a[s & 1][f], acc[f][nf], 0, 0, 0);
      if (s + 1 < KSTEPS) {
#pragma unroll
        for (int f = 0; f < G::MF_WAVE; ++f) {
          __builtin_amdgcn_sched_group_barrier(0x100, 1, 0);
          __builtin_amdgcn_sched_group_barrier(0x008, 1, 0);
        }
        if constexpr (NFW > 1) __builtin_amdgcn_sched_group_barrier(0x008, G::MF_WAVE * (NFW - 1), 0);
      }
      __builtin_amdgcn_sched_barrier(0);
    }

#pragma unroll
    for (int f = 0; f < G::MF_WAVE; ++f)
#pragma unroll
      for (int nf = 0; nf < NFW; ++nf) {
        const int p = (wm * G::MF_WAVE + f) * 16 + l15;
        const int ch = (2 * (NFW * wn + nf) + (lh >> 1)) ^ stage_key(p);
        *reinterpret_cast<bf16x4*>(ostage + p * C64 + ch * 8 + (lh & 1) * 4) =
            __builtin_convertvector(acc[f][nf], bf16x4);
      }
    __syncthreads();
    {
      const int n = t / tiles_per_img;
      const int r0 = (t - n * tiles_per_img) * R;
      const int rows = min(R, H - r0);
      const int chunks = rows * W * (C64 / 8);
      full_prev = chunks == G::STORES_PER_THREAD * G::NT;
      bf16* dst = y + (((int64_t)n * H + r0) * W) * C64;
      for (int i = threadIdx.x; i < chunks; i += G::NT) {
        const int sp = i >> 3;
        const bf16x8 v = *reinterpret_cast<const bf16x8*>(ostage + sp * C64 + (((i & 7) ^ stage_key(sp)) << 3));
        *reinterpret_cast<bf16x8*>(dst + i * 8) = v;
        if constexpr (MOM)
#pragma unroll
          for (int j = 0; j < 8; ++j) {
            const float fv = (float)v[j];
            s8[j] += fv;
            q8[j] = fmaf(fv, fv, q8[j]);
          }
      }
    }
    cur ^= 1;
  }

  if constexpr (MOM) {
#pragma unroll
    for (int j = 0; j < 8; ++j) {
#pragma unroll
      for (int off = 8; off < 64; off <<= 1) {
        s8[j] += __shfl_xor(s8[j], off, 64);
        q8[j] += __shfl_xor(q8[j], off, 64);
      }
    }
    if (lane < 8)
#pragma unroll
      for (int j = 0; j < 8; ++j) {
        atomicAdd(&mred[8 * lane + j], s8[j]);
        atomicAdd(&mred[C64 + 8 * lane + j], q8[j]);
      }
    __syncthreads();
    if (threadIdx.x < 2 * C64) {
      const int mo = threadIdx.x / C64, ch = threadIdx.x % C64;
      part[((int64_t)mo * gridDim.x + blockIdx.x) * C64 + ch] = mred[mo * C64 + ch];
    }
  }
}

template <int W, int R, int NW, bool MOM>
void launch_nw(const at::Tensor& x, const at::Tensor& wk, at::Tensor& y, float* part, double* zs, int H,
               int tiles, int tpi, int grid, hipStream_t stream) {
  using G = HaloGeo<W, R, NW>;
  static_assert(G::SMEM_BYTES <= 160 * 1024, "LDS budget");
  auto kern = conv3x3_c64_kernel<W, R, NW, MOM>;
  hipLaunchKernelGGL(kern, dim3(grid), dim3(G::NT), 0, stream,
                     reinterpret_cast<const bf16*>(x.data_ptr()), reinterpret_cast<const bf16*>(wk.data_ptr()),
                     reinterpret_cast<bf16*>(y.data_ptr()), part, zs, H, tiles, tpi);
}

template <int W, int R, bool MOM>
void launch(const at::Tensor& x, const at::Tensor& wk, at::Tensor& y, float* part, double* zs, int H,
            int tiles, int tpi, int grid, hipStream_t stream) {
  launch_nw<W, R, 4, MOM>(x, wk, y, part, zs, H, tiles, tpi, grid, stream);
}

}

std::vector<at::Tensor> conv3x3_c64(const at::Tensor& x, const at::Tensor& wmat, bool moments) {
  constexpr int W = 56, R = 4;
  TORCH_CHECK(x.is_cuda() && x.scalar_type() == at::kBFloat16 && x.dim() == 4, "conv3x3_c64: bf16 NCHW-shaped x");
  TORCH_CHECK(x.size(1) == C64 && x.size(3) == W && x.is_contiguous(at::MemoryFormat::ChannelsLast),
              "conv3x3_c64: x must be [N, 64, H, 56] channels_last");
  TORCH_CHECK(wmat.scalar_type() == at::kBFloat16 && wmat.is_contiguous() && wmat.size(0) == C64 &&
                  wmat.size(1) == 9 * C64, "conv3x3_c64: wmat must be contiguous [64, 576] bf16");
  const int64_t n = x.size(0), H = x.size(2);
  const int tpi = (int)((H + R - 1) / R);
  const int64_t tiles64 = n * tpi;
  TORCH_CHECK(tiles64 < (1 << 30), "conv3x3_c64: too many tiles");
  const int tiles = (int)tiles64;
  auto y = at::empty({n * H * W, C64}, x.options());
  auto stream = at::hip::getCurrentHIPStream();
  at::Tensor mom;
  if (tiles == 0) return {y, at::zeros({moments ? 2 * C64 + 1 : 0}, x.options().dtype(at::kDouble))};
  int dev = 0, cus = 256;
  DMP_HIP_CHECK(hipGetDevice(&dev));
  DMP_HIP_CHECK(hipDeviceGetAttribute(&cus, hipDeviceAttributeMultiprocessorCount, dev));
  const int grid = std::min(tiles, cus);
  if (moments) {
    mom = at::empty({2 * C64 + 1}, x.options().dtype(at::kDouble));
    auto part = at::empty({2, grid, C64}, x.options().dtype(at::kFloat));
    launch<W, R, true>(x, wmat, y, part.data_ptr<float>(), moments_zero_target(mom.data_ptr<double>(), grid),
                       (int)H, tiles, tpi, grid, stream);
    bn_reduce_partials_launch(part.data_ptr<float>(), grid, C64, mom.data_ptr<double>(),
                              (double)(n * H * W), stream);
  } else {
    mom = at::empty({0}, x.options().dtype(at::kDouble));
    launch<W, R, false>(x, wmat, y, nullptr, nullptr, (int)H, tiles, tpi, grid, stream);
  }
  DMP_HIP_CHECK(hipGetLastError());
  return {y, mom};
}

}
```

### distributed_model_parallel_amd/_native.py

```python
from __future__ import annotations

import contextlib
import os
import threading
from types import ModuleType
from typing import Optional

import torch

_lock = threading.Lock()
_mod: Optional[ModuleType] = None
_err: Optional[BaseException] = None
_tried = False


def _load() -> Optional[ModuleType]:
    global _mod, _err, _tried
    with _lock:
        if _tried:
            return _mod
        _tried = True
        if os.environ.get("DMP_DISABLE_NATIVE") == "1":
            _err = RuntimeError("DMP_DISABLE_NATIVE=1")
            return None
        try:
            so = os.environ.get("DMP_NATIVE_SO")
            if so:
                import importlib.util
                import sys
                spec = importlib.util.spec_from_file_location(f"{__package__}._C", so)
                _mod = importlib.util.module_from_spec(spec)
                spec.loader.exec_module(_mod)
                sys.modules[f"{__package__}._C"] = _mod
                return _mod
            from . import _C
            _mod = _C
        except ImportError as e:
            _err = e
            _mod = None
        return _mod


_PROBE = None


def native() -> Optional[ModuleType]:
    if _PROBE is not None:
        return _PROBE
    return _load()


def available() -> bool:
    return _load() is not None


def require(what: str = "this operation") -> ModuleType:
    if _PROBE is not None:
        return _PROBE
    m = _load()
    if m is None:
        raise RuntimeError(
            f"distributed_model_parallel_amd native extension is required for {what} but could "
            f"not be loaded ({_err!r}). Build it with `python csrc/build.py` "
            f"(or `python -c 'import __graft_entry__ as g; g.build()'`).")
    return m


FEATURES = {
    "igemm": "every native 3x3 conv (ops/conv_igemm.py) -> MIOpen",
    "halo3": "halo-tiled 3x3 convs of layers 1-2 (conv3x3_halo.hip, conv3x3_c128.hip)",
    "xl_conv3": "256x256 implicit GEMM for layer-3/4 3x3 convs (gemm_xl.hip conv_xl; kernels gemm_xl_w4.hip, gemm_xl_nt8.hip)",
    "xl_conv": "256x256 GEMM for wide 1x1 convs (gemm_xl.hip gemm_xl_conv; kernels gemm_xl_w4.hip, gemm_xl_nt8.hip, gemm_xl_x2.hip)",
    "tn_xl": "ping-pong TN weight gradients of wide 1x1 convs and of the ViT linears",
    "xl_linear": "ViT MLP / attention projection on the fused-epilogue ping-pong GEMM -> hipBLASLt + GELU / add passes",
    "fuse_drop_path": "stochastic depth's per-sample scale in the proj / fc2 GEMM store and the backward side pass "
                      "(gemm_xl bias_res_scale, rowscale_bias_grad) -> the plain GEMM path + a scale and an add pass",
    "compact_shortcut": "stride-2 shortcut gradient kept compact (no zero-filled tensor)",
    "fuse_bn_bwd": "BN backward reductions in the consumer's data-gradient epilogue (BnBwdSlot)",
    "fuse_stem_pool": "stem BN apply + ReLU inside the max-pool (forward and backward)",
    "stem_halo": "halo-tiled stem kernels (stem_halo.hip) -> row-tap implicit GEMM",
    "rowtap_stem": "row-tap stem implicit GEMM (stem.hip) -> MIOpen",
    "bn_fold": "bottleneck bn3 folded through conv3 (ops/bn_fold.py) -> conv + BN apply passes",
    "bn_fold_ds": "downsample conv + BN folded into the same GEMM as bn3 (ops/bn_fold.py) -> separate shortcut",
    "fuse_bn_gram": "the bn3 fold's Gram a2^T a2 formed inside bn2's apply pass (bn_apply_gram.hip) "
                    "-> the apply pass + a TN GEMM over its output",
    "fuse_stem_wgrad": "stem BN backward apply folded into the stem weight gradient (ops/fused.py) "
                       "-> the apply pass + one weight gradient",
    "fuse_stem_pool_wgrad": "stem pool / ReLU backward formed inside the stem weight-gradient kernel "
                            "(stem_halo.hip stem_halo_wgrad_pool) -> maxpool2d_bn_backward + two stem_halo_wgrad",
    "fuse_ema": "weight EMA updated inside the flat optimizers' step kernels (ops/optim.py ema_decay) "
                "-> the step kernel + a lerp_ pass over the masters",
    "gpu_augment": "crop / resize / flip / normalise / cast / layout of a uint8 batch in one kernel (augment.hip, "
                   "data/gpu_augment.py) -> the PyTorch composition, sample by sample",
    "async_wgrad": "weight gradients on a side stream beside the data-gradient chain (ops/wgrad_stream.py) "
                   "-> inline on the compute stream",
}
_disabled_cache: Optional[frozenset] = None


def disabled(feature: str) -> bool:
    global _disabled_cache
    if _disabled_cache is None:
        names = {f.strip() for f in os.environ.get("DMP_DISABLE", "").split(",") if f.strip()}
        unknown = names - set(FEATURES)
        if unknown:
            raise ValueError(f"DMP_DISABLE: unknown feature(s) {sorted(unknown)}; known: {sorted(FEATURES)}")
        _disabled_cache = frozenset(names)
    if feature not in FEATURES:
        raise KeyError(feature)
    return feature in _disabled_cache


_REFERENCE = False


@contextlib.contextmanager
def reference_mode():
    global _REFERENCE
    prev, _REFERENCE = _REFERENCE, True
    try:
        yield
    finally:
        _REFERENCE = prev


def gpu_path(t: torch.Tensor) -> bool:
    if _REFERENCE:
        return False
    if t.is_cuda:
        require(f"GPU op on {t.device}")
        return True
    return False
```

### distributed_model_parallel_amd/ops/conv_igemm.py

```python
from __future__ import annotations

import contextlib


from typing import Optional, Tuple

import torch
import torch.nn as nn
import torch.nn.functional as F

from .. import _native
from . import wgrad_stream, wt_cache

_STATS = {"native": 0, "torch": 0}
ENABLED = not _native.disabled("igemm")
NATIVE_BWD = False


def set_generic_backward(on: bool) -> None:
    global NATIVE_BWD
    NATIVE_BWD = bool(on)


def _capturing() -> bool:
    return torch.cuda.is_current_stream_capturing()


_XL_WGRAD = not _native.disabled("xl_conv3")
_STATS["xl_wgrad"] = 0


def _xl_wgrad_ok(cin: int, kh: int, kw: int, rows: int) -> bool:
    return _XL_WGRAD and cin % 256 == 0 and kh == kw and kh > 1

_XL3 = not _native.disabled("xl_conv3")
_STATS["xl_fwd"] = 0
_STATS["xl_dgrad"] = 0
_STATS["xl_bnbwd"] = 0


_MIOPEN_FWD = True
_STATS["miopen_fwd"] = 0


_HALO3 = not _native.disabled("halo3")
_STATS["halo_fwd"] = 0
_STATS["halo_dgrad"] = 0


def _halo_kind(cin: int, cout: int, kh: int, kw: int, stride: int, pad: int, h: int, wdt: int) -> int:
    if not (_HALO3 and cin == cout and kh == 3 and kw == 3 and stride == 1 and pad == 1):
        return 0
    if cin == 64 and wdt == 56:
        return 64
    if cin == 128 and wdt == 28 and h % 4 == 0:
        return 128
    return 0


def _halo_conv(C, kind: int):
    return C.conv3x3_c64 if kind == 64 else C.conv3x3_c128


_STATS["halo_dgrad_s2"] = 0


def _halo_dgrad_s2_ok(cin: int, cout: int, kh: int, kw: int, stride: int, pad: int, h: int, w: int) -> bool:
    return (_HALO3 and cin == 128 and cout == 128 and kh == 3 and kw == 3 and stride == 2 and pad == 1
            and w == 56 and h % 8 == 0)


_STATS["halo_wgrad"] = 0


def _halo_wgrad_ok(C, cin: int, cout: int, kh: int, kw: int, stride: int, pad: int, h: int, w: int) -> bool:
    return (kh == 3 and kw == 3 and stride in (1, 2) and pad == 1 and cin == cout and h == w
            and h % stride == 0 and C.wgrad3x3_supported(cin, h // stride, w // stride, stride))


def _miopen_fwd(cout: int, kh: int) -> bool:
    return _MIOPEN_FWD and kh > 1 and not _xl_fwd(cout, kh, kh)


_XL_N128 = True


def _xl_fwd(cout: int, kh: int, kw: int) -> bool:
    return _XL3 and (cout >= 256 or (cout == 128 and _XL_N128)) and kh == kw and kh > 1


def _xl_dgrad(cin: int, kh: int, kw: int, stride: int) -> bool:
    return _XL3 and cin >= 256 and stride == 1 and kh == kw and kh > 1


_STATS["xl_dgrad_s2"] = 0
_PHASE_TAPS = ((1,), (2, 0))


def _xl_dgrad_s2(cin: int, cout: int, kh: int, kw: int, stride: int, pad: int, h: int, w: int) -> bool:
    return (_XL3 and cin % 256 == 0 and cout % 64 == 0 and kh == 3 and kw == 3 and stride == 2 and pad == 1
            and h % 2 == 0 and w % 2 == 0)


def _phase_weights(weight: torch.Tensor):
    cin = weight.shape[1]
    w4 = weight.permute(1, 2, 3, 0)
    out = []
    for py in (0, 1):
        for px in (0, 1):
            taps = [w4[:, ky, kx] for ky in _PHASE_TAPS[py] for kx in _PHASE_TAPS[px]]
            out.append(torch.stack(taps, 1).reshape(cin, -1))
    return out


def _out_size(h: int, k: int, s: int, p: int) -> int:
    return (h + 2 * p - k) // s + 1


def _native_ok(x: torch.Tensor, w: torch.Tensor, groups: int, dilation) -> bool:
    if not ENABLED or not _native.gpu_path(x):
        return False
    return (groups == 1 and tuple(dilation) == (1, 1) and x.dtype == torch.bfloat16
            and w.dtype == torch.bfloat16 and x.dim() == 4 and x.shape[1] % 64 == 0
            and w.shape[0] % 64 == 0 and x.is_contiguous(memory_format=torch.channels_last))


def _wmat(w: torch.Tensor) -> torch.Tensor:
    return w.permute(0, 2, 3, 1).reshape(w.shape[0], -1)


class _ConvIGFn(torch.autograd.Function):
    @staticmethod
    def forward(ctx, x, weight, stride, pad, moments, bn_slot=None):
        C = _native.require("conv_igemm")
        n, cin, h, w = x.shape
        cout, _, kh, kw = weight.shape
        ho, wo = _out_size(h, kh, stride, pad), _out_size(w, kw, stride, pad)
        mode = "moments" if moments else "store"
        y4 = None
        if moments is None:
            y4 = F.conv2d(x, weight, None, stride, pad)
            y2, mom = None, None
        elif _halo_kind(cin, cout, kh, kw, stride, pad, h, w):
            _STATS["halo_fwd"] += 1
            y2, mom = _halo_conv(C, _halo_kind(cin, cout, kh, kw, stride, pad, h, w))(
                x, _wmat(weight).contiguous(), moments)
            if not moments:
                mom = None
        elif _xl_fwd(cout, kh, kw):
            _STATS["xl_fwd"] += 1
            y2, mom = C.conv_xl(x, _wmat(weight), kh, kw, stride, pad, ho, wo, mode)
            if not moments:
                mom = None
        else:
            y2, mom = C.conv_nt(x, _wmat(weight), kh, kw, stride, pad, ho, wo, mode=mode)
        ctx.save_for_backward(x, weight)
        ctx.geo = (stride, pad, ho, wo)
        ctx.bn_slot = bn_slot if (bn_slot is not None and _xl_dgrad(cin, kh, kw, stride)) else None
        if ctx.bn_slot is not None:
            bn_slot.consumers += 1
        if mom is None:
            mom = torch.empty(0, device=x.device, dtype=torch.float64)
        ctx.mark_non_differentiable(mom)
        ctx.set_materialize_grads(False)
        if y4 is not None:
            return y4, mom
        return y2.view(n, ho, wo, cout).permute(0, 3, 1, 2), mom

    @staticmethod
    def backward(ctx, dy, _dmom):
        if dy is None:
            return (None,) * 6
        x, weight = ctx.saved_tensors
        C = _native.require("conv_igemm backward")
        stride, pad, ho, wo = ctx.geo
        n, cin, h, w = x.shape
        cout, _, kh, kw = weight.shape
        dy = dy.to(x.dtype).contiguous(memory_format=torch.channels_last)
        dx = dw = None
        bs, ctx.bn_slot = ctx.bn_slot, None
        hk = _halo_kind(cin, cout, kh, kw, stride, pad, h, w)
        if ctx.needs_input_grad[0] and hk:
            wfl = wt_cache.flipped(weight)
            _STATS["halo_dgrad"] += 1
            dx2, _ = _halo_conv(C, hk)(dy, wfl, False)
            dx = dx2.view(n, h, w, cin).permute(0, 3, 1, 2)
        elif ctx.needs_input_grad[0] and _xl_dgrad(cin, kh, kw, stride):
            wfl = wt_cache.flipped(weight)
            _STATS["xl_dgrad"] += 1
            if bs is not None and bs.consumers == 1 and bs.x2 is not None:
                _STATS["xl_bnbwd"] += 1
                inv, bw, bb = (bs.invstd, bs.w32, bs.b32) if bs.y2 is None else (None, None, None)
                dx2, sums = C.conv_xl(dy, wfl, kh, kw, 1, kh - 1 - pad, h, w, "bnbwd", bn_x=bs.x2, bn_y=bs.y2,
                                      mean=bs.mean, invstd=inv, weight=bw, bias=bb)
                dx = dx2.view(n, h, w, cin).permute(0, 3, 1, 2)
                bs.park(dx, sums[: 2 * cin])
            else:
                dx2, _ = C.conv_xl(dy, wfl, kh, kw, 1, kh - 1 - pad, h, w, "store")
                dx = dx2.view(n, h, w, cin).permute(0, 3, 1, 2)
        elif ctx.needs_input_grad[0] and _halo_dgrad_s2_ok(cin, cout, kh, kw, stride, pad, h, w):
            _STATS["halo_dgrad_s2"] += 1
            wt = weight.permute(1, 2, 3, 0).reshape(cin, -1).contiguous()
            dx = C.conv3x3_c128_dgrad_s2(dy, wt).view(n, h, w, cin).permute(0, 3, 1, 2)
        elif ctx.needs_input_grad[0] and _xl_dgrad_s2(cin, cout, kh, kw, stride, pad, h, w):
            _STATS["xl_dgrad_s2"] += 1
            dx2 = C.conv_xl_dgrad_s2(dy, _phase_weights(weight), h, w)
            dx = dx2.view(n, h, w, cin).permute(0, 3, 1, 2)
        if ctx.needs_input_grad[1] and _halo_wgrad_ok(C, cin, cout, kh, kw, stride, pad, h, w):
            _STATS["halo_wgrad"] += 1
            with wgrad_stream.side(weight, dy, x):
                dw = C.wgrad3x3(dy, x, stride)
                if not weight.is_contiguous(memory_format=torch.channels_last):
                    dw = dw.contiguous()
        if ctx.needs_input_grad[1] and dw is None and _xl_wgrad_ok(cin, kh, kw, n * ho * wo):
            _STATS["xl_wgrad"] += 1
            with wgrad_stream.side(weight, dy, x):
                dy2 = dy.permute(0, 2, 3, 1).reshape(-1, cout)
                g = C.conv_wgrad_xl(dy2, x, kh, kw, stride, pad, ho, wo, weight.dtype)
                dw = g.view(cout, kh, kw, cin).permute(0, 3, 1, 2)
                if not weight.is_contiguous(memory_format=torch.channels_last):
                    dw = dw.contiguous()
        generic = NATIVE_BWD or _capturing()
        nat_d = ctx.needs_input_grad[0] and dx is None and generic
        nat_w = ctx.needs_input_grad[1] and dw is None and generic
        want_d = ctx.needs_input_grad[0] and not nat_d and dx is None
        want_w = ctx.needs_input_grad[1] and not nat_w and dw is None
        if want_d or want_w:
            with (wgrad_stream.side(weight, dy, x) if not want_d else contextlib.nullcontext()):
                dx_l, dw_l, _ = torch.ops.aten.convolution_backward(
                    dy, x, weight, None, [stride, stride], [pad, pad], [1, 1], False, [0, 0], 1,
                    [want_d, want_w, False])
            if want_d:
                dx = dx_l
            if want_w:
                dw = dw_l
        if nat_d:
            wt = weight.permute(1, 2, 3, 0).reshape(cin, -1).contiguous()
            dx2, _ = C.conv_nt(dy, wt, kh, kw, stride, pad, h, w, transposed=True)
            dx = dx2.view(n, h, w, cin).permute(0, 3, 1, 2)
        if nat_w:
            with wgrad_stream.side(weight, dy, x):
                dy2 = dy.permute(0, 2, 3, 1).reshape(-1, cout)
                g = C.conv_wgrad(dy2, x, kh, kw, stride, pad, ho, wo, weight.dtype)
                dw = g.view(cout, kh, kw, cin).permute(0, 3, 1, 2)
                if not weight.is_contiguous(memory_format=torch.channels_last):
                    dw = dw.contiguous()
        return dx, dw, None, None, None, None


def conv2d_igemm(x: torch.Tensor, weight: torch.Tensor, stride: int = 1, padding: int = 0,
                 moments: bool = False, groups: int = 1,
                 dilation=(1, 1)) -> Tuple[torch.Tensor, Optional[torch.Tensor]]:
    if _native_ok(x, weight, groups, dilation) and _miopen_fwd(weight.shape[0], weight.shape[2]) and \
            not _capturing() and not \
            _halo_kind(x.shape[1], weight.shape[0], weight.shape[2], weight.shape[3], stride, padding, x.shape[2],
                       x.shape[3]):
        _STATS["miopen_fwd"] += 1
        geo = (x.shape[1], weight.shape[0], weight.shape[2], weight.shape[3], stride, padding, x.shape[2],
               x.shape[3])
        if torch.is_grad_enabled() and (weight.requires_grad or x.requires_grad) and (
                _halo_wgrad_ok(_native.native(), *geo) or _halo_dgrad_s2_ok(*geo) or _xl_dgrad_s2(*geo)):
            y, _ = _ConvIGFn.apply(x, weight, stride, padding, None, None)
            return y, None
        return F.conv2d(x, weight, None, stride, padding, dilation, groups), None
    if _native_ok(x, weight, groups, dilation):
        _STATS["native"] += 1
        bn_slot = getattr(x, "_dmp_bnbwd", None) if torch.is_grad_enabled() else None
        y, mom = _ConvIGFn.apply(x, weight, stride, padding, moments, bn_slot)
        return y, (mom if moments else None)
    _STATS["torch"] += 1
    return F.conv2d(x, weight, None, stride, padding, dilation, groups), None


class ConvIG2d(nn.Conv2d):

    def __init__(self, cin: int, cout: int, kernel_size: int, stride: int = 1, padding: int = 0,
                 device=None, dtype=None):
        super().__init__(cin, cout, kernel_size, stride=stride, padding=padding, bias=False,
                         device=device, dtype=dtype)

    def forward(self, x: torch.Tensor) -> torch.Tensor:
        return conv2d_igemm(x, self.weight, self.stride[0], self.padding[0], False,
                            self.groups, self.dilation)[0]

    def forward_with_moments(self, x: torch.Tensor):
        return conv2d_igemm(x, self.weight, self.stride[0], self.padding[0], True,
                            self.groups, self.dilation)
```

Before: 18650 images/sec.

## Fuse BN+ReLU backward reductions into halo 3x3 data-gradient epilogues

Adds a BN-backward epilogue to the halo 3x3 conv kernels (c64, c128, and the c128 stride-2 dgrad). The epilogue loads the BN input, masks the gradient by the ReLU sign recomputed from the BN affine, and accumulates sum dz and sum dz*(x-mean) in-kernel. This replaces a separate gradient write, re-read and moments pass for bn1 in layers 1-2. The cost is extra register and LDS pressure and an extra global read inside persistent MFMA kernels, which could slow the main loop.

```diff
diff --git a/csrc/api.h b/csrc/api.h
--- a/csrc/api.h
+++ b/csrc/api.h
@@ -100,8 +100,20 @@
 std::vector<at::Tensor> conv3x3_c128(const at::Tensor& x, const at::Tensor& wmat, bool moments);
 bool conv3x3_c128_supported(int64_t c, int64_t h, int64_t w);
 at::Tensor conv3x3_c128_dgrad_s2(const at::Tensor& dy, const at::Tensor& wt);
+std::vector<at::Tensor> conv3x3_c128_bnbwd(const at::Tensor& x, const at::Tensor& wmat, const at::Tensor& bn_x,
+                                           const at::Tensor& mean, const at::Tensor& invstd,
+                                           const c10::optional<at::Tensor>& weight,
+                                           const c10::optional<at::Tensor>& bias);
+std::vector<at::Tensor> conv3x3_c128_dgrad_s2_bnbwd(const at::Tensor& dy, const at::Tensor& wt, const at::Tensor& bn_x,
+                                                    const at::Tensor& mean, const at::Tensor& invstd,
+                                                    const c10::optional<at::Tensor>& weight,
+                                                    const c10::optional<at::Tensor>& bias);
 
 std::vector<at::Tensor> conv3x3_c64(const at::Tensor& x, const at::Tensor& wmat, bool moments);
+std::vector<at::Tensor> conv3x3_c64_bnbwd(const at::Tensor& x, const at::Tensor& wmat, const at::Tensor& bn_x,
+                                          const at::Tensor& mean, const at::Tensor& invstd,
+                                          const c10::optional<at::Tensor>& weight,
+                                          const c10::optional<at::Tensor>& bias);
 
 std::vector<at::Tensor> dwconv3x3_forward(const at::Tensor& x, const at::Tensor& w, int64_t stride,
                                           bool moments);
diff --git a/csrc/bindings.cpp b/csrc/bindings.cpp
--- a/csrc/bindings.cpp
+++ b/csrc/bindings.cpp
@@ -164,6 +164,20 @@
   m.def("conv3x3_c128_dgrad_s2", &dmp::conv3x3_c128_dgrad_s2, py::arg("dy"), py::arg("wt"),
         "data gradient of a 3x3/s2/p1 128->128 conv (dy 28 wide) as its four stride phases on the halo kernel; "
         "wt = W.permute(1, 2, 3, 0) as [128, 1152]; returns dx [N*2H*56, 128]",
+        py::call_guard<py::gil_scoped_release>());
+  m.def("conv3x3_c64_bnbwd", &dmp::conv3x3_c64_bnbwd, py::arg("x"), py::arg("wmat"), py::arg("bn_x"), py::arg("mean"),
+        py::arg("invstd"), py::arg("weight") = py::none(), py::arg("bias") = py::none(),
+        "conv3x3_c64 as the data gradient arriving at a training-mode BN+ReLU with input bn_x [N*H*W, 64]: "
+        "returns (dz = gradient masked by the BN's forward sign, fp64 [129] = sum dz, sum dz (bn_x - mean), rows)",
+        py::call_guard<py::gil_scoped_release>());
+  m.def("conv3x3_c128_bnbwd", &dmp::conv3x3_c128_bnbwd, py::arg("x"), py::arg("wmat"), py::arg("bn_x"),
+        py::arg("mean"), py::arg("invstd"), py::arg("weight") = py::none(), py::arg("bias") = py::none(),
+        "conv3x3_c128 with the BN-backward epilogue of conv3x3_c64_bnbwd; returns (dz [N*H*W, 128], fp64 [257])",
+        py::call_guard<py::gil_scoped_release>());
+  m.def("conv3x3_c128_dgrad_s2_bnbwd", &dmp::conv3x3_c128_dgrad_s2_bnbwd, py::arg("dy"), py::arg("wt"),
+        py::arg("bn_x"), py::arg("mean"), py::arg("invstd"), py::arg("weight") = py::none(),
+        py::arg("bias") = py::none(),
+        "conv3x3_c128_dgrad_s2 with the BN-backward epilogue; bn_x [N*2H*56, 128]; returns (dz, fp64 [257])",
         py::call_guard<py::gil_scoped_release>());
   m.def("conv3x3_c128_supported", &dmp::conv3x3_c128_supported, py::arg("C"), py::arg("H"), py::arg("W"));
   m.def("conv_xl_dgrad_s2", &dmp::conv_xl_dgrad_s2, py::arg("dy"), py::arg("wph"), py::arg("hi"), py::arg("wi"),
diff --git a/csrc/conv/conv3x3_c128.hip b/csrc/conv/conv3x3_c128.hip
--- a/csrc/conv/conv3x3_c128.hip
+++ b/csrc/conv/conv3x3_c128.hip
@@ -175,12 +175,27 @@
   __syncthreads();
 }
 
-template <bool MOM, bool PH>
+enum { EPI_STORE = 0, EPI_MOMENTS = 1, EPI_BNBWD = 2 };
+
+struct HaloBnOps {
+  const bf16* x;
+  const float* mean;
+  const float* invstd;
+  const float* weight;
+  const float* bias;
+};
+
+constexpr int CHUNKS_PER_THREAD = (OUT_PIX * 8 + NT - 1) / NT;
+
+template <int EPI, bool PH>
 __global__ __launch_bounds__(NT, 1) void conv3x3_c128_kernel(
     const bf16* __restrict__ x, const bf16* __restrict__ wk, bf16* __restrict__ y, float* __restrict__ part,
-    double* zsums, int H, int tiles) {
+    double* zsums, int H, int tiles, HaloBnOps bn) {
   using G = Geo<PH>;
-  __shared__ __attribute__((aligned(1024))) char smem[G::SMEM];
+  constexpr bool MOM = EPI == EPI_MOMENTS, BNB = EPI == EPI_BNBWD;
+  constexpr bool SUMS = MOM || BNB;
+  static_assert(G::SMEM + 3 * CB * 4 <= 160 * 1024, "LDS budget");
+  __shared__ __attribute__((aligned(1024))) char smem[G::SMEM + (EPI == EPI_BNBWD ? 3 * CB * 4 : 0)];
   f32x4* scr = reinterpret_cast<f32x4*>(smem + G::SCR_OFF);
   bf16* ostage = reinterpret_cast<bf16*>(smem + G::STAGE_OFF);
   float* mred = reinterpret_cast<float*>(smem + G::MRED_OFF);
@@ -191,7 +206,7 @@
   const int cb = (int)blockIdx.x >= half ? 1 : 0;
   const int rb = (int)blockIdx.x - cb * half;
   const int tpi = H / R;
-  if constexpr (MOM) {
+  if constexpr (SUMS) {
     zero_moments(zsums, 2 * CO);
     if (threadIdx.x < 2 * CB) mred[threadIdx.x] = 0.f;
   }
@@ -226,6 +241,34 @@
   float s8[8], q8[8];
 #pragma unroll
   for (int j = 0; j < 8; ++j) s8[j] = q8[j] = 0.f;
+  float* bnc = reinterpret_cast<float*>(smem + G::SMEM);
+  if constexpr (BNB) {
+    if (threadIdx.x < CB) {
+      const int c = CB * cb + threadIdx.x;
+      const float mu = bn.mean[c], sc = bn.weight[c] * bn.invstd[c];
+      bnc[threadIdx.x] = sc;
+      bnc[CB + threadIdx.x] = bn.bias[c] - mu * sc;
+      bnc[2 * CB + threadIdx.x] = mu;
+    }
+    __syncthreads();
+    if constexpr (!PH)
+#pragma unroll
+      for (int nf = 0; nf < 2; ++nf)
+#pragma unroll
+        for (int s = 0; s < KSTEPS; ++s) asm volatile("" : "+v"(bw[nf][s]));
+  }
+  uint32_t boff[CHUNKS_PER_THREAD];
+  if constexpr (BNB) {
+#pragma unroll
+    for (int k = 0; k < CHUNKS_PER_THREAD; ++k) {
+      const int ik = (int)threadIdx.x + k * NT;
+      const int i = ik < OUT_PIX * 8 ? ik : (int)threadIdx.x;
+      const int sp = i >> 3;
+      const int m = sp / W, q = sp - m * W;
+      const int pix = PH ? 2 * m * (2 * W) + 2 * q : sp;
+      boff[k] = (uint32_t)(pix * CO + CB * cb + (i & 7) * 8);
+    }
+  }
   int cur = 0;
   bool stored_prev = false;
   for (int t = t_begin; t < t_end; ++t) {
@@ -260,14 +303,81 @@
           }
       }
     };
+    const int64_t tile_el = (PH ? ((int64_t)n * (2 * H) + 2 * r0) * (2 * W) : ((int64_t)n * H + r0) * W) * CO;
+    auto load_bnx = [&](bf16x8 (&xr)[CHUNKS_PER_THREAD], int py, int px) __attribute__((always_inline)) {
+      const bf16* src = bn.x + tile_el + (py * 2 * W + px) * CO;
+#pragma unroll
+      for (int k = 0; k < CHUNKS_PER_THREAD; ++k) asm volatile("" : "+v"(boff[k]));
+#pragma unroll
+      for (int k = 0; k < CHUNKS_PER_THREAD; ++k)
+        if (!PH || (int)threadIdx.x + k * NT < OUT_PIX * 8) xr[k] = *reinterpret_cast<const bf16x8*>(src + boff[k]);
+    };
+    auto store_stage_bn = [&](bf16x8 (&xr)[CHUNKS_PER_THREAD], int py, int px) __attribute__((always_inline)) {
+      bf16* dst = y + tile_el + (py * 2 * W + px) * CO;
+#pragma unroll
+      for (int k = 0; k < CHUNKS_PER_THREAD; ++k) asm volatile("" : "+v"(boff[k]));
+      const f32x4* cf = reinterpret_cast<const f32x4*>(bnc) + 2 * (threadIdx.x & 7);
+      const f32x4 c4[6] = {cf[0], cf[1], cf[CB / 4], cf[CB / 4 + 1], cf[CB / 2], cf[CB / 2 + 1]};
+      float bsc[8], bsh[8], bmu[8];
+#pragma unroll
+      for (int j = 0; j < 8; ++j) {
+        bsc[j] = c4[j >> 2][j & 3];
+        bsh[j] = c4[2 + (j >> 2)][j & 3];
+        bmu[j] = c4[4 + (j >> 2)][j & 3];
+      }
+      auto mask_chunk = [&](int k, int i, bool live) __attribute__((always_inline)) {
+        const int sp = i >> 3;
+        bf16x8 v = *reinterpret_cast<const bf16x8*>(ostage + sp * CB + (((i & 7) ^ stage_key(sp)) << 3));
+#pragma unroll
+        for (int j = 0; j < 8; ++j) {
+          const float xv = (float)xr[k][j];
+          const bool on = live && fmaf(xv, bsc[j], bsh[j]) > 0.f;
+          const float dz = on ? (float)v[j] : 0.f;
+          v[j] = (bf16)dz;
+          s8[j] += dz;
+          q8[j] = fmaf(dz, xv - bmu[j], q8[j]);
+        }
+        xr[k] = v;
+      };
+      if constexpr (PH) {
+#pragma unroll
+        for (int k = 0; k < CHUNKS_PER_THREAD; ++k) {
+          const int i = (int)threadIdx.x + k * NT;
+          if (i < OUT_PIX * 8) {
+            mask_chunk(k, i, true);
+            *reinterpret_cast<bf16x8*>(dst + boff[k]) = xr[k];
+          }
+        }
+      } else {
+#pragma unroll
+        for (int k = 0; k < CHUNKS_PER_THREAD; ++k) {
+          const int ik = (int)threadIdx.x + k * NT;
+          mask_chunk(k, ik < OUT_PIX * 8 ? ik : (int)threadIdx.x, ik < OUT_PIX * 8);
+        }
+#pragma unroll
+        for (int k = 0; k < CHUNKS_PER_THREAD; ++k) asm volatile("" : "+v"(xr[k]));
+#pragma unroll
+        for (int k = 0; k < CHUNKS_PER_THREAD; ++k)
+          if ((int)threadIdx.x + k * NT < OUT_PIX * 8) *reinterpret_cast<bf16x8*>(dst + boff[k]) = xr[k];
+      }
+    };
     auto phase = [&](auto pyc, auto pxc) __attribute__((always_inline)) {
       constexpr int PY = decltype(pyc)::value, PX = decltype(pxc)::value;
+      constexpr int py = PY < 0 ? 0 : PY, px = PX < 0 ? 0 : PX;
       f32x4 acc[MF][2];
 #pragma unroll
       for (int f = 0; f < MF; ++f) acc[f][0] = acc[f][1] = f32x4{0.f, 0.f, 0.f, 0.f};
-      sweep<PH, PY, PX>(acc, bw, hb, qb, kt, lchunk);
-      exchange_to_stage(acc, scr, ostage, wkh, wn, lane, l15, lh);
-      store_stage(PY < 0 ? 0 : PY, PX < 0 ? 0 : PX);
+      if constexpr (BNB) {
+        bf16x8 xr[CHUNKS_PER_THREAD];
+        load_bnx(xr, py, px);
+        sweep<PH, PY, PX>(acc, bw, hb, qb, kt, lchunk);
+        exchange_to_stage(acc, scr, ostage, wkh, wn, lane, l15, lh);
+        store_stage_bn(xr, py, px);
+      } else {
+        sweep<PH, PY, PX>(acc, bw, hb, qb, kt, lchunk);
+        exchange_to_stage(acc, scr, ostage, wkh, wn, lane, l15, lh);
+        store_stage(py, px);
+      }
     };
     using I0 = std::integral_constant<int, 0>;
     using I1 = std::integral_constant<int, 1>;
@@ -284,7 +394,7 @@
     cur ^= 1;
   }
 
-  if constexpr (MOM) {
+  if constexpr (SUMS) {
 #pragma unroll
     for (int j = 0; j < 8; ++j)
 #pragma unroll
@@ -344,17 +454,17 @@
   if (moments) {
     mom = at::empty({2 * CO + 1}, x.options().dtype(at::kDouble));
     auto part = at::empty({2, half, CO}, x.options().dtype(at::kFloat));
-    hipLaunchKernelGGL((conv3x3_c128_kernel<true, false>), dim3(grid), dim3(NT), 0, stream,
+    hipLaunchKernelGGL((conv3x3_c128_kernel<EPI_MOMENTS, false>), dim3(grid), dim3(NT), 0, stream,
                        reinterpret_cast<const bf16*>(x.data_ptr()), reinterpret_cast<const bf16*>(wmat.data_ptr()),
                        reinterpret_cast<bf16*>(y.data_ptr()), part.data_ptr<float>(),
-                       moments_zero_target(mom.data_ptr<double>(), half), (int)H, tiles);
+                       moments_zero_target(mom.data_ptr<double>(), half), (int)H, tiles, HaloBnOps{});
     bn_reduce_partials_launch(part.data_ptr<float>(), half, CO, mom.data_ptr<double>(), (double)(n * H * W),
                               stream);
   } else {
     mom = at::empty({0}, x.options().dtype(at::kDouble));
-    hipLaunchKernelGGL((conv3x3_c128_kernel<false, false>), dim3(grid), dim3(NT), 0, stream,
+    hipLaunchKernelGGL((conv3x3_c128_kernel<EPI_STORE, false>), dim3(grid), dim3(NT), 0, stream,
                        reinterpret_cast<const bf16*>(x.data_ptr()), reinterpret_cast<const bf16*>(wmat.data_ptr()),
-                       reinterpret_cast<bf16*>(y.data_ptr()), nullptr, nullptr, (int)H, tiles);
+                       reinterpret_cast<bf16*>(y.data_ptr()), nullptr, nullptr, (int)H, tiles, HaloBnOps{});
   }
   DMP_HIP_CHECK(hipGetLastError());
   return {y, mom};
@@ -376,11 +486,73 @@
   if (tiles == 0) return dx;
   auto stream = at::hip::getCurrentHIPStream();
   const int half = grid_half(tiles);
-  hipLaunchKernelGGL((conv3x3_c128_kernel<false, true>), dim3(2 * half), dim3(NT), 0, stream,
+  hipLaunchKernelGGL((conv3x3_c128_kernel<EPI_STORE, true>), dim3(2 * half), dim3(NT), 0, stream,
                      reinterpret_cast<const bf16*>(dy.data_ptr()), reinterpret_cast<const bf16*>(wt.data_ptr()),
-                     reinterpret_cast<bf16*>(dx.data_ptr()), nullptr, nullptr, (int)H, tiles);
+                     reinterpret_cast<bf16*>(dx.data_ptr()), nullptr, nullptr, (int)H, tiles, HaloBnOps{});
   DMP_HIP_CHECK(hipGetLastError());
   return dx;
 }
 
-}
+namespace {
+
+template <bool PH>
+std::vector<at::Tensor> c128_bnbwd(const char* who, const at::Tensor& x, const at::Tensor& wmat,
+                                   const at::Tensor& bn_x, const at::Tensor& mean, const at::Tensor& invstd,
+                                   const c10::optional<at::Tensor>& weight,
+                                   const c10::optional<at::Tensor>& bias) {
+  TORCH_CHECK(x.is_cuda() && x.scalar_type() == at::kBFloat16 && x.dim() == 4, who, ": bf16 NCHW-shaped input");
+  TORCH_CHECK(conv3x3_c128_supported(x.size(1), x.size(2), x.size(3)) &&
+                  x.is_contiguous(at::MemoryFormat::ChannelsLast),
+              who, ": input must be [N, 128, H % 4 == 0, 28] channels_last");
+  check_wmat(wmat, who);
+  TORCH_CHECK(wmat.device() == x.device(), who, ": device mismatch");
+  const int64_t n = x.size(0), H = x.size(2);
+  const int64_t rows = n * H * W * (PH ? 4 : 1);
+  const int64_t tiles64 = n * (H / R);
+  TORCH_CHECK(tiles64 < (1 << 30) && rows < (1LL << 31), who, ": too large");
+  TORCH_CHECK(bn_x.scalar_type() == at::kBFloat16 && bn_x.is_contiguous() && bn_x.device() == x.device() &&
+                  bn_x.numel() == rows * CO, who, ": bn_x must be contiguous [rows of the result, 128] bf16");
+  const auto fopt = x.options().dtype(at::kFloat);
+  auto vec = [&](const at::Tensor& t, const char* name) {
+    TORCH_CHECK(t.scalar_type() == at::kFloat && t.is_contiguous() && t.numel() == CO && t.device() == x.device(),
+                who, ": ", name, " must be contiguous fp32 [128]");
+    return t.data_ptr<float>();
+  };
+  const at::Tensor wv = weight.has_value() && weight->defined() ? *weight : at::ones({CO}, fopt);
+  const at::Tensor bv = bias.has_value() && bias->defined() ? *bias : at::zeros({CO}, fopt);
+  const int tiles = (int)tiles64;
+  auto y = at::empty({rows, CO}, x.options());
+  if (tiles == 0) return {y, at::zeros({2 * CO + 1}, x.options().dtype(at::kDouble))};
+  HaloBnOps bn{reinterpret_cast<const bf16*>(bn_x.data_ptr()), vec(mean, "mean"), vec(invstd, "invstd"),
+               vec(wv, "weight"), vec(bv, "bias")};
+  auto stream = at::hip::getCurrentHIPStream();
+  const int half = grid_half(tiles);
+  auto sums = at::empty({2 * CO + 1}, x.options().dtype(at::kDouble));
+  auto part = at::empty({2, half, CO}, fopt);
+  hipLaunchKernelGGL((conv3x3_c128_kernel<EPI_BNBWD, PH>), dim3(2 * half), dim3(NT), 0, stream,
+                     reinterpret_cast<const bf16*>(x.data_ptr()), reinterpret_cast<const bf16*>(wmat.data_ptr()),
+                     reinterpret_cast<bf16*>(y.data_ptr()), part.data_ptr<float>(),
+                     moments_zero_target(sums.data_ptr<double>(), half), (int)H, tiles, bn);
+  bn_reduce_partials_launch(part.data_ptr<float>(), half, CO, sums.data_ptr<double>(), (double)rows, stream);
+  DMP_HIP_CHECK(hipGetLastError());
+  return {y, sums};
+}
+
+}
+
+std::vector<at::Tensor> conv3x3_c128_bnbwd(const at::Tensor& x, const at::Tensor& wmat, const at::Tensor& bn_x,
+                                           const at::Tensor& mean, const at::Tensor& invstd,
+                                           const c10::optional<at::Tensor>& weight,
+                                           const c10::optional<at::Tensor>& bias) {
+  return c128_bnbwd<false>("conv3x3_c128_bnbwd", x, wmat, bn_x, mean, invstd, weight, bias);
+}
+
+std::vector<at::Tensor> conv3x3_c128_dgrad_s2_bnbwd(const at::Tensor& dy, const at::Tensor& wt,
+                                                    const at::Tensor& bn_x, const at::Tensor& mean,
+                                                    const at::Tensor& invstd,
+                                                    const c10::optional<at::Tensor>& weight,
+                                                    const c10::optional<at::Tensor>& bias) {
+  return c128_bnbwd<true>("conv3x3_c128_dgrad_s2_bnbwd", dy, wt, bn_x, mean, invstd, weight, bias);
+}
+
+}
diff --git a/csrc/conv/conv3x3_halo.hip b/csrc/conv/conv3x3_halo.hip
--- a/csrc/conv/conv3x3_halo.hip
+++ b/csrc/conv/conv3x3_halo.hip
@@ -101,19 +101,32 @@
   }
 }
 
-template <int W, int R, int NW, bool MOM>
+enum { EPI_STORE = 0, EPI_MOMENTS = 1, EPI_BNBWD = 2 };
+
+struct HaloBnOps {
+  const bf16* x;
+  const float* mean;
+  const float* invstd;
+  const float* weight;
+  const float* bias;
+};
+
+template <int W, int R, int NW, int EPI>
 __global__ __launch_bounds__(64 * NW, 1) void conv3x3_c64_kernel(
     const bf16* __restrict__ x, const bf16* __restrict__ wk, bf16* __restrict__ y, float* __restrict__ part,
-    double* zsums, int H, int tiles, int tiles_per_img) {
+    double* zsums, int H, int tiles, int tiles_per_img, HaloBnOps bn) {
   using G = HaloGeo<W, R, NW>;
   constexpr int NFW = G::NFW;
+  constexpr bool MOM = EPI == EPI_MOMENTS, BNB = EPI == EPI_BNBWD;
+  constexpr bool SUMS = MOM || BNB;
+  static_assert(!BNB || G::STORES_EXACT, "EPI_BNBWD keeps one bn.x register set per output chunk");
   __shared__ __attribute__((aligned(1024))) char smem[G::SMEM_BYTES];
   bf16* ostage = reinterpret_cast<bf16*>(smem + 2 * G::BUF_BYTES);
   float* mred = reinterpret_cast<float*>(smem + 2 * G::BUF_BYTES + G::OUT_PIX * C64 * 2);
   const int lane = threadIdx.x & 63, wave = threadIdx.x >> 6;
   const int wm = wave & 1, wn = wave >> 1;
   const int l15 = lane & 15, lh = lane >> 4;
-  if constexpr (MOM) {
+  if constexpr (SUMS) {
     zero_moments(zsums, 2 * C64);
     if (threadIdx.x < 2 * C64) mred[threadIdx.x] = 0.f;
   }
@@ -146,6 +159,27 @@
   float s8[8], q8[8];
 #pragma unroll
   for (int j = 0; j < 8; ++j) s8[j] = q8[j] = 0.f;
+  float bsc[8], bsh[8], bmu[8];
+  if constexpr (BNB) {
+    const int c0 = 8 * (threadIdx.x & 7);
+    float wv[8], bv[8], iv[8];
+#pragma unroll
+    for (int j = 0; j < 8; ++j) {
+      wv[j] = bn.weight[c0 + j];
+      bv[j] = bn.bias[c0 + j];
+      iv[j] = bn.invstd[c0 + j];
+      bmu[j] = bn.mean[c0 + j];
+    }
+#pragma unroll
+    for (int j = 0; j < 8; ++j) {
+      bsc[j] = wv[j] * iv[j];
+      bsh[j] = bv[j] - bmu[j] * bsc[j];
+    }
+#pragma unroll
+    for (int nf = 0; nf < NFW; ++nf)
+#pragma unroll
+      for (int s = 0; s < KSTEPS; ++s) asm volatile("" : "+v"(bw[nf][s]));
+  }
   int cur = 0;
   bool full_prev = false;
   for (int t = t_begin; t < t_end; ++t) {
@@ -160,6 +194,19 @@
     raw_barrier();
     if (t + 1 < t_end) halo_issue<W, R, NW>(x, smem + (cur ^ 1) * G::BUF_BYTES, t + 1, H, tiles_per_img, wave, lane, hs);
     const char* hb = smem + cur * G::BUF_BYTES;
+
+    bf16x8 xr[BNB ? G::STORES_PER_THREAD : 1];
+    if constexpr (BNB) {
+      const int n = t / tiles_per_img;
+      const int r0 = (t - n * tiles_per_img) * R;
+      const int chunks = min(R, H - r0) * W * (C64 / 8);
+      const bf16* src = bn.x + (((int64_t)n * H + r0) * W) * C64;
+#pragma unroll
+      for (int k = 0; k < G::STORES_PER_THREAD; ++k) {
+        const int i = (int)threadIdx.x + k * G::NT;
+        xr[k] = *reinterpret_cast<const bf16x8*>(src + (i < chunks ? i : (int)threadIdx.x) * 8);
+      }
+    }
 
     f32x4 acc[G::MF_WAVE][NFW];
 #pragma unroll
@@ -214,6 +261,32 @@
       const int chunks = rows * W * (C64 / 8);
       full_prev = chunks == G::STORES_PER_THREAD * G::NT;
       bf16* dst = y + (((int64_t)n * H + r0) * W) * C64;
+      if constexpr (BNB) {
+#pragma unroll
+        for (int k = 0; k < G::STORES_PER_THREAD; ++k) {
+          const int i = (int)threadIdx.x + k * G::NT;
+          const bool live = i < chunks;
+          const int sp = i >> 3;
+          bf16x8 v = *reinterpret_cast<const bf16x8*>(ostage + sp * C64 + (((i & 7) ^ stage_key(sp)) << 3));
+#pragma unroll
+          for (int j = 0; j < 8; ++j) {
+            const float xv = (float)xr[k][j];
+            const bool on = live && fmaf(xv, bsc[j], bsh[j]) > 0.f;
+            const float dz = on ? (float)v[j] : 0.f;
+            v[j] = (bf16)dz;
+            s8[j] += dz;
+            q8[j] = fmaf(dz, xv - bmu[j], q8[j]);
+          }
+          xr[k] = v;
+        }
+#pragma unroll
+        for (int k = 0; k < G::STORES_PER_THREAD; ++k) asm volatile("" : "+v"(xr[k]));
+#pragma unroll
+        for (int k = 0; k < G::STORES_PER_THREAD; ++k) {
+          const int i = (int)threadIdx.x + k * G::NT;
+          if (i < chunks) *reinterpret_cast<bf16x8*>(dst + i * 8) = xr[k];
+        }
+      } else
       for (int i = threadIdx.x; i < chunks; i += G::NT) {
         const int sp = i >> 3;
         const bf16x8 v = *reinterpret_cast<const bf16x8*>(ostage + sp * C64 + (((i & 7) ^ stage_key(sp)) << 3));
@@ -230,7 +303,7 @@
     cur ^= 1;
   }
 
-  if constexpr (MOM) {
+  if constexpr (SUMS) {
 #pragma unroll
     for (int j = 0; j < 8; ++j) {
 #pragma unroll
@@ -253,21 +326,21 @@
   }
 }
 
-template <int W, int R, int NW, bool MOM>
+template <int W, int R, int NW, int EPI>
 void launch_nw(const at::Tensor& x, const at::Tensor& wk, at::Tensor& y, float* part, double* zs, int H,
-               int tiles, int tpi, int grid, hipStream_t stream) {
+               int tiles, int tpi, int grid, hipStream_t stream, const HaloBnOps& bn) {
   using G = HaloGeo<W, R, NW>;
   static_assert(G::SMEM_BYTES <= 160 * 1024, "LDS budget");
-  auto kern = conv3x3_c64_kernel<W, R, NW, MOM>;
+  auto kern = conv3x3_c64_kernel<W, R, NW, EPI>;
   hipLaunchKernelGGL(kern, dim3(grid), dim3(G::NT), 0, stream,
                      reinterpret_cast<const bf16*>(x.data_ptr()), reinterpret_cast<const bf16*>(wk.data_ptr()),
-                     reinterpret_cast<bf16*>(y.data_ptr()), part, zs, H, tiles, tpi);
-}
-
-template <int W, int R, bool MOM>
+                     reinterpret_cast<bf16*>(y.data_ptr()), part, zs, H, tiles, tpi, bn);
+}
+
+template <int W, int R, int EPI>
 void launch(const at::Tensor& x, const at::Tensor& wk, at::Tensor& y, float* part, double* zs, int H,
-            int tiles, int tpi, int grid, hipStream_t stream) {
-  launch_nw<W, R, 4, MOM>(x, wk, y, part, zs, H, tiles, tpi, grid, stream);
+            int tiles, int tpi, int grid, hipStream_t stream, const HaloBnOps& bn = HaloBnOps{}) {
+  launch_nw<W, R, 4, EPI>(x, wk, y, part, zs, H, tiles, tpi, grid, stream, bn);
 }
 
 }
@@ -295,16 +368,62 @@
   if (moments) {
     mom = at::empty({2 * C64 + 1}, x.options().dtype(at::kDouble));
     auto part = at::empty({2, grid, C64}, x.options().dtype(at::kFloat));
-    launch<W, R, true>(x, wmat, y, part.data_ptr<float>(), moments_zero_target(mom.data_ptr<double>(), grid),
+    launch<W, R, EPI_MOMENTS>(x, wmat, y, part.data_ptr<float>(), moments_zero_target(mom.data_ptr<double>(), grid),
                        (int)H, tiles, tpi, grid, stream);
     bn_reduce_partials_launch(part.data_ptr<float>(), grid, C64, mom.data_ptr<double>(),
                               (double)(n * H * W), stream);
   } else {
     mom = at::empty({0}, x.options().dtype(at::kDouble));
-    launch<W, R, false>(x, wmat, y, nullptr, nullptr, (int)H, tiles, tpi, grid, stream);
+    launch<W, R, EPI_STORE>(x, wmat, y, nullptr, nullptr, (int)H, tiles, tpi, grid, stream);
   }
   DMP_HIP_CHECK(hipGetLastError());
   return {y, mom};
 }
 
-}
+std::vector<at::Tensor> conv3x3_c64_bnbwd(const at::Tensor& x, const at::Tensor& wmat, const at::Tensor& bn_x,
+                                          const at::Tensor& mean, const at::Tensor& invstd,
+                                          const c10::optional<at::Tensor>& weight,
+                                          const c10::optional<at::Tensor>& bias) {
+  constexpr int W = 56, R = 4;
+  TORCH_CHECK(x.is_cuda() && x.scalar_type() == at::kBFloat16 && x.dim() == 4,
+              "conv3x3_c64_bnbwd: bf16 NCHW-shaped x");
+  TORCH_CHECK(x.size(1) == C64 && x.size(3) == W && x.is_contiguous(at::MemoryFormat::ChannelsLast),
+              "conv3x3_c64_bnbwd: x must be [N, 64, H, 56] channels_last");
+  TORCH_CHECK(wmat.scalar_type() == at::kBFloat16 && wmat.is_contiguous() && wmat.size(0) == C64 &&
+                  wmat.size(1) == 9 * C64 && wmat.device() == x.device(),
+              "conv3x3_c64_bnbwd: wmat must be contiguous [64, 576] bf16");
+  const int64_t n = x.size(0), H = x.size(2);
+  TORCH_CHECK(bn_x.scalar_type() == at::kBFloat16 && bn_x.is_contiguous() && bn_x.device() == x.device() &&
+                  bn_x.numel() == n * H * W * C64, "conv3x3_c64_bnbwd: bn_x must be contiguous [N*H*W, 64] bf16");
+  const auto fopt = x.options().dtype(at::kFloat);
+  auto vec = [&](const at::Tensor& t, const char* name) {
+    TORCH_CHECK(t.scalar_type() == at::kFloat && t.is_contiguous() && t.numel() == C64 && t.device() == x.device(),
+                "conv3x3_c64_bnbwd: ", name, " must be contiguous fp32 [64]");
+    return t.data_ptr<float>();
+  };
+  const at::Tensor wv = weight.has_value() && weight->defined() ? *weight : at::ones({C64}, fopt);
+  const at::Tensor bv = bias.has_value() && bias->defined() ? *bias : at::zeros({C64}, fopt);
+  const int tpi = (int)((H + R - 1) / R);
+  const int64_t tiles64 = n * tpi;
+  TORCH_CHECK(tiles64 < (1 << 30), "conv3x3_c64_bnbwd: too many tiles");
+  const int tiles = (int)tiles64;
+  auto y = at::empty({n * H * W, C64}, x.options());
+  if (tiles == 0) return {y, at::zeros({2 * C64 + 1}, x.options().dtype(at::kDouble))};
+  HaloBnOps bn{reinterpret_cast<const bf16*>(bn_x.data_ptr()), vec(mean, "mean"), vec(invstd, "invstd"),
+               vec(wv, "weight"), vec(bv, "bias")};
+  auto stream = at::hip::getCurrentHIPStream();
+  int dev = 0, cus = 256;
+  DMP_HIP_CHECK(hipGetDevice(&dev));
+  DMP_HIP_CHECK(hipDeviceGetAttribute(&cus, hipDeviceAttributeMultiprocessorCount, dev));
+  const int grid = std::min(tiles, cus);
+  auto sums = at::empty({2 * C64 + 1}, x.options().dtype(at::kDouble));
+  auto part = at::empty({2, grid, C64}, fopt);
+  launch<W, R, EPI_BNBWD>(x, wmat, y, part.data_ptr<float>(), moments_zero_target(sums.data_ptr<double>(), grid),
+                          (int)H, tiles, tpi, grid, stream, bn);
+  bn_reduce_partials_launch(part.data_ptr<float>(), grid, C64, sums.data_ptr<double>(), (double)(n * H * W),
+                            stream);
+  DMP_HIP_CHECK(hipGetLastError());
+  return {y, sums};
+}
+
+}
diff --git a/distributed_model_parallel_amd/_native.py b/distributed_model_parallel_amd/_native.py
--- a/distributed_model_parallel_amd/_native.py
+++ b/distributed_model_parallel_amd/_native.py
@@ -84,6 +84,8 @@
     "bn_fold_ds": "downsample conv + BN folded into the same GEMM as bn3 (ops/bn_fold.py) -> separate shortcut",
     "fuse_bn_gram": "the bn3 fold's Gram a2^T a2 formed inside bn2's apply pass (bn_apply_gram.hip) "
                     "-> the apply pass + a TN GEMM over its output",
+    "fuse_halo_bnbwd": "bn1's backward reductions in the epilogue of the halo 3x3 data gradients of layers 1-2 "
+                       "(conv3x3_*_bnbwd, BnBwdSlot) -> the plain data gradient + bn_backward_moments",
     "fuse_stem_wgrad": "stem BN backward apply folded into the stem weight gradient (ops/fused.py) "
                        "-> the apply pass + one weight gradient",
     "fuse_stem_pool_wgrad": "stem pool / ReLU backward formed inside the stem weight-gradient kernel "
diff --git a/distributed_model_parallel_amd/ops/conv_igemm.py b/distributed_model_parallel_amd/ops/conv_igemm.py
--- a/distributed_model_parallel_amd/ops/conv_igemm.py
+++ b/distributed_model_parallel_amd/ops/conv_igemm.py
@@ -68,6 +68,30 @@
 def _halo_dgrad_s2_ok(cin: int, cout: int, kh: int, kw: int, stride: int, pad: int, h: int, w: int) -> bool:
     return (_HALO3 and cin == 128 and cout == 128 and kh == 3 and kw == 3 and stride == 2 and pad == 1
             and w == 56 and h % 8 == 0)
+
+
+_FUSE_HALO_BNBWD = not _native.disabled("fuse_halo_bnbwd")
+_HALO_BNBWD_ALL = ("c64", "c128", "c128s2")
+_HALO_BNBWD_KINDS = _HALO_BNBWD_ALL
+_STATS["halo_bnbwd"] = 0
+
+
+def set_halo_bnbwd_kinds(kinds) -> None:
+    global _HALO_BNBWD_KINDS
+    kinds = tuple(kinds)
+    if not set(kinds) <= set(_HALO_BNBWD_ALL):
+        raise ValueError(f"unknown halo bnbwd kind in {kinds!r}; known: {_HALO_BNBWD_ALL}")
+    _HALO_BNBWD_KINDS = kinds
+
+
+def _halo_bnbwd_kind(cin: int, cout: int, kh: int, kw: int, stride: int, pad: int, h: int, w: int):
+    if not _FUSE_HALO_BNBWD:
+        return None
+    hk = _halo_kind(cin, cout, kh, kw, stride, pad, h, w)
+    kind = {64: "c64", 128: "c128"}.get(hk)
+    if kind is None and _halo_dgrad_s2_ok(cin, cout, kh, kw, stride, pad, h, w):
+        kind = "c128s2"
+    return kind if kind in _HALO_BNBWD_KINDS else None
 
 
 _STATS["halo_wgrad"] = 0
@@ -156,7 +180,9 @@
             y2, mom = C.conv_nt(x, _wmat(weight), kh, kw, stride, pad, ho, wo, mode=mode)
         ctx.save_for_backward(x, weight)
         ctx.geo = (stride, pad, ho, wo)
-        ctx.bn_slot = bn_slot if (bn_slot is not None and _xl_dgrad(cin, kh, kw, stride)) else None
+        ctx.bn_slot = bn_slot if (bn_slot is not None and (
+            _xl_dgrad(cin, kh, kw, stride)
+            or _halo_bnbwd_kind(cin, cout, kh, kw, stride, pad, h, w) is not None)) else None
         if ctx.bn_slot is not None:
             bn_slot.consumers += 1
         if mom is None:
@@ -180,11 +206,21 @@
         dx = dw = None
         bs, ctx.bn_slot = ctx.bn_slot, None
         hk = _halo_kind(cin, cout, kh, kw, stride, pad, h, w)
+        hb = None
+        if bs is not None and bs.consumers == 1 and bs.x2 is not None and bs.y2 is None:
+            hb = _halo_bnbwd_kind(cin, cout, kh, kw, stride, pad, h, w)
         if ctx.needs_input_grad[0] and hk:
             wfl = wt_cache.flipped(weight)
             _STATS["halo_dgrad"] += 1
-            dx2, _ = _halo_conv(C, hk)(dy, wfl, False)
-            dx = dx2.view(n, h, w, cin).permute(0, 3, 1, 2)
+            if hb is not None:
+                _STATS["halo_bnbwd"] += 1
+                fn = C.conv3x3_c64_bnbwd if hk == 64 else C.conv3x3_c128_bnbwd
+                dx2, sums = fn(dy, wfl, bs.x2, bs.mean, bs.invstd, bs.w32, bs.b32)
+                dx = dx2.view(n, h, w, cin).permute(0, 3, 1, 2)
+                bs.park(dx, sums[: 2 * cin])
+            else:
+                dx2, _ = _halo_conv(C, hk)(dy, wfl, False)
+                dx = dx2.view(n, h, w, cin).permute(0, 3, 1, 2)
         elif ctx.needs_input_grad[0] and _xl_dgrad(cin, kh, kw, stride):
             wfl = wt_cache.flipped(weight)
             _STATS["xl_dgrad"] += 1
@@ -201,7 +237,13 @@
         elif ctx.needs_input_grad[0] and _halo_dgrad_s2_ok(cin, cout, kh, kw, stride, pad, h, w):
             _STATS["halo_dgrad_s2"] += 1
             wt = weight.permute(1, 2, 3, 0).reshape(cin, -1).contiguous()
-            dx = C.conv3x3_c128_dgrad_s2(dy, wt).view(n, h, w, cin).permute(0, 3, 1, 2)
+            if hb is not None:
+                _STATS["halo_bnbwd"] += 1
+                dx2, sums = C.conv3x3_c128_dgrad_s2_bnbwd(dy, wt, bs.x2, bs.mean, bs.invstd, bs.w32, bs.b32)
+                dx = dx2.view(n, h, w, cin).permute(0, 3, 1, 2)
+                bs.park(dx, sums[: 2 * cin])
+            else:
+                dx = C.conv3x3_c128_dgrad_s2(dy, wt).view(n, h, w, cin).permute(0, 3, 1, 2)
         elif ctx.needs_input_grad[0] and _xl_dgrad_s2(cin, cout, kh, kw, stride, pad, h, w):
             _STATS["xl_dgrad_s2"] += 1
             dx2 = C.conv_xl_dgrad_s2(dy, _phase_weights(weight), h, w)
```

Measured after the change: 18750 images/sec (median of 6 runs). About the same (+0.5%).
